# PositronicsLab/Moby

Hardware: AMD Instinct MI355X
Metric: lcp_rows_per_sec (higher is better)
Workload: dtype f64

## Files before the change

moby_amd/csrc/mh_lcp_wave.h:

```cpp
#pragma once
#include "mh_wave.h"
#include "../../include/moby_hip.h"

namespace mh {

enum { LP_SETUP = 0, LP_GATHER, LP_LU, LP_GEMV, LP_RANDMIN, LP_VERIFY, LP_LEMKE, LP_COUNT };
__shared__ unsigned long long g_lcp_prof[LP_COUNT];
__shared__ int g_lcp_prof_on;
#ifdef MH_PROFILE_BUILD
MH_DEV unsigned long long lp_tick() { return g_lcp_prof_on ? __builtin_amdgcn_s_memtime() : 0ull; }
MH_DEV void lp_tock(int ph, unsigned long long t0) { if (g_lcp_prof_on) { const unsigned long long d = __builtin_amdgcn_s_memtime() - t0; if (lane_id() == 0) g_lcp_prof[ph] += d; } }
#else
MH_DEV unsigned long long lp_tick() { return 0ull; }
MH_DEV void lp_tock(int, unsigned long long) {}
#endif

struct Trace {
  int32_t* buf; int cap; int len;
  MH_DEV void push(int32_t v) { if (buf && len < cap && lane_id() == 0) buf[len] = v; len++; }
};

#define MH_DBL_EPS 2.220446049250313e-16
#define MH_NEAR_ZERO 1.4901161193847656e-08
#define MH_SFMIN 2.2250738585072014e-308

struct DenseLds {
  const double* M; int n;
  MH_DEV double at_row(int c) const { const int l = lane_id(); return (l < n) ? M[l + n * c] : 0.0; }
  MH_DEV double diag() const { const int l = lane_id(); return (l < n) ? M[l + n * l] : 0.0; }
  MH_DEV double offdiag_max() const {
    const int lane = lane_id();
    double m = 0.0;
    if (lane < n)
      for (int c = 0; c < n; c++) {
        const double a = fabs(M[lane + n * c]);
        if (c != lane && a > m) m = a;
      }
    return wave_max(m);
  }
};

template <class MatT>
MH_DEV double mat_at(const MatT& M, int c, double lam) {
  const double m = M.at_row(c);
  return (lane_id() == c) ? m + lam : m;
}

MH_DEV int lu_solve_wave(int k, double* A, double& b)
{
  const int lane = lane_id();
  for (int j = 0; j < k; j++) {
    const bool mine = (lane >= j) && (lane < k);
    double a = mine ? fabs(A[lane + k * j]) : -1.0;
    double amax; int jp;
    argmax_first(a, mine, amax, jp);
    if (!(amax != 0.0)) return j + 1;
    if (jp != j) {
      if (lane < k) { double t0 = A[j + k * lane], t1 = A[jp + k * lane]; A[j + k * lane] = t1; A[jp + k * lane] = t0; }
      double bj = read_lane(b, j), bjp = read_lane(b, jp);
      if (lane == j) b = bjp; else if (lane == jp) b = bj;
      wave_sync();
    }
    if (j < k - 1) {
      const double piv = A[j + k * j];
      if (lane > j && lane < k) {
        double l = A[lane + k * j];
        if (fabs(piv) >= MH_SFMIN) { const double r = 1.0 / piv; l = l * r; } else l = l / piv;
        A[lane + k * j] = l;
        for (int c0 = j + 1; c0 < k; c0 += 8) {
          double a[8], u[8];
#pragma unroll
          for (int t = 0; t < 8; t++) {
            const int c = (c0 + t < k) ? c0 + t : k - 1;
            a[t] = A[lane + k * c]; u[t] = A[j + k * c];
          }
#pragma unroll
          for (int t = 0; t < 8; t++)
            if (c0 + t < k) A[lane + k * (c0 + t)] = a[t] - l * u[t];
        }
      }
      wave_sync();
    }
  }
  for (int kk = 0; kk < k; kk++) {
    const double bk = read_lane(b, kk);
    if (lane > kk && lane < k) b = b - bk * A[lane + k * kk];
  }
  for (int kk = k - 1; kk >= 0; kk--) {
    if (lane == kk) b = b / A[kk + k * kk];
    const double bk = read_lane(b, kk);
    if (lane < kk) b = b - bk * A[lane + k * kk];
  }
  return 0;
}

MH_DEV int lu_solve_wave_hbm(int k, double* A, double& b)
{
  constexpr int PB = 8;
  const int lane = lane_id();
  const bool valid = lane < k;
  int prow = lane;
  for (int j0 = 0; j0 < k; j0 += PB) {
    const int nb = (k - j0 < PB) ? k - j0 : PB;
    double p[PB];
#pragma unroll
    for (int c = 0; c < PB; c++) p[c] = (valid && c < nb) ? A[prow + k * (j0 + c)] : 0.0;
#pragma unroll
    for (int jj = 0; jj < PB; jj++) {
      if (jj < nb) {
        const int j = j0 + jj;
        const bool mine = (lane >= j) && valid;
        double amax; int jp;
        argmax_first(mine ? fabs(p[jj]) : -1.0, mine, amax, jp);
        if (!(amax != 0.0)) return j + 1;
        if (jp != j) {
#pragma unroll
          for (int c = 0; c < PB; c++) { const double vj = read_lane(p[c], j), vp = read_lane(p[c], jp); if (lane == j) p[c] = vp; else if (lane == jp) p[c] = vj; }
          { const double vj = read_lane(b, j), vp = read_lane(b, jp); if (lane == j) b = vp; else if (lane == jp) b = vj; }
          { const int rj = read_lane(prow, j), rp = read_lane(prow, jp); if (lane == j) prow = rp; else if (lane == jp) prow = rj; }
        }
        if (j < k - 1) {
          const double piv = read_lane(p[jj], j);
          const bool below = (lane > j) && valid;
          if (below) { double l = p[jj]; if (fabs(piv) >= MH_SFMIN) { const double r = 1.0 / piv; l = l * r; } else l = l / piv; p[jj] = l; }
#pragma unroll
          for (int c = 0; c < PB; c++) if (c > jj && c < nb) { const double u = read_lane(p[c], j); if (below) p[c] = p[c] - p[jj] * u; }
        }
      }
    }
#pragma unroll
    for (int c = 0; c < PB; c++) if (valid && c < nb) A[prow + k * (j0 + c)] = p[c];
    for (int cb = j0 + nb; cb < k; cb += PB) {
      double a[PB];
#pragma unroll
      for (int u = 0; u < PB; u++) a[u] = (valid && cb + u < k) ? A[prow + k * (cb + u)] : 0.0;
#pragma unroll
      for (int u = 0; u < PB; u++) {
#pragma unroll
        for (int s2 = 0; s2 < PB; s2++) if (s2 < nb) { const double us = read_lane(a[u], j0 + s2); if (lane > j0 + s2 && valid) a[u] = a[u] - p[s2] * us; }
      }
#pragma unroll
      for (int u = 0; u < PB; u++) if (valid && cb + u < k) A[prow + k * (cb + u)] = a[u];
    }
  }
  wave_sync();
  for (int kb = 0; kb < k; kb += PB) {
    double l[PB];
#pragma unroll
    for (int u = 0; u < PB; u++) l[u] = (valid && kb + u < k) ? A[prow + k * (kb + u)] : 0.0;
#pragma unroll
    for (int u = 0; u < PB; u++) if (kb + u < k) { const double bk = read_lane(b, kb + u); if (lane > kb + u && valid) b = b - bk * l[u]; }
  }
  for (int ke = k; ke > 0; ke -= PB) {
    const int kb = (ke - PB > 0) ? ke - PB : 0;
    double uu[PB];
#pragma unroll
    for (int u = 0; u < PB; u++) uu[u] = (valid && kb + u < ke) ? A[prow + k * (kb + u)] : 1.0;
#pragma unroll
    for (int u = PB - 1; u >= 0; u--) if (kb + u < ke) {
      const int kk = kb + u;
      if (lane == kk) b = b / uu[u];
      const double bk = read_lane(b, kk);
      if (lane < kk) b = b - bk * uu[u];
    }
  }
  return 0;
}

MH_DEV int rand_min_wave(double v, uint64_t mask, double tol, WaveRand& rng, double& val, bool& tie)
{
  const int lane = lane_id();
  const bool in = (mask >> lane) & 1ull;
  double vmin; int imin;
  if (popc(mask) <= 4) {
    uint64_t m = mask;
    imin = ctz(m); m &= m - 1;
    vmin = read_lane(v, imin);
    while (m) { const int i = ctz(m); m &= m - 1; const double x = read_lane(v, i); if (x < vmin) { vmin = x; imin = i; } }
  } else argmin_first(v, in, vmin, imin);
  const uint64_t qm = ballot(in && lane != imin && v < vmin + tol);
  const int cnt = 1 + popc(qm);
  tie = tie || cnt > 1;
  const int rv = rng.next();
  const int r = (cnt == 1) ? 0 : rv % cnt;
  const int chosen = (r == 0) ? imin : nth_set_bit(qm, r - 1);
  val = read_lane(v, chosen);
  return chosen;
}

MH_DEV double norm_reg(double offmax, double dii, bool valid, double lam) {
  double d = valid ? fabs(dii + lam) : 0.0;
  double m = wave_max(d);
  return (m > offmax) ? m : offmax;
}

struct LuScratch { double* small; int ka; double* big; };

template <int K>
MH_DEV int lu_small(const double* A, double& b)
{
  double a[K][K], x[K];
#pragma unroll
  for (int c = 0; c < K; c++)
#pragma unroll
    for (int r = 0; r < K; r++) a[r][c] = A[r + K * c];
#pragma unroll
  for (int r = 0; r < K; r++) x[r] = read_lane(b, r);
#pragma unroll
  for (int j = 0; j < K; j++) {
    int jp = j; double amax = fabs(a[j][j]);
#pragma unroll
    for (int i = j + 1; i < K; i++) { const double v = fabs(a[i][j]); if (v > amax) { amax = v; jp = i; } }
    jp = uni(jp);
    if (ballot(!(amax != 0.0)) != 0ull) return j + 1;
#pragma unroll
    for (int i = j + 1; i < K; i++)
      if (jp == i) {
#pragma unroll
        for (int c = 0; c < K; c++) { const double t = a[j][c]; a[j][c] = a[i][c]; a[i][c] = t; }
        const double t = x[j]; x[j] = x[i]; x[i] = t;
      }
    if (j < K - 1) {
      const double piv = a[j][j];
      const bool big = fabs(piv) >= MH_SFMIN;
      const double r = 1.0 / piv;
#pragma unroll
      for (int i = j + 1; i < K; i++) {
        const double l = big ? a[i][j] * r : a[i][j] / piv;
        a[i][j] = l;
#pragma unroll
        for (int c = j + 1; c < K; c++) a[i][c] = a[i][c] - l * a[j][c];
      }
    }
  }
#pragma unroll
  for (int kk = 0; kk < K; kk++)
#pragma unroll
    for (int i = kk + 1; i < K; i++) x[i] = x[i] - x[kk] * a[i][kk];
#pragma unroll
  for (int kk = K - 1; kk >= 0; kk--) {
    x[kk] = x[kk] / a[kk][kk];
#pragma unroll
    for (int i = 0; i < kk; i++) x[i] = x[i] - x[kk] * a[i][kk];
  }
  const int lane = lane_id();
  double out = 0.0;
#pragma unroll
  for (int r = 0; r < K; r++) out = (lane == r) ? x[r] : out;
  b = out;
  return 0;
}

#ifndef MH_COLCACHE
#define MH_COLCACHE 4
#endif
template <bool REGLU, class MatT>
MH_DEV int gather_and_solve(const MatT& M, double lam, uint64_t nbmask, int k, bool is_nb, int pos, double qi, double* A, double& b,
                            double (&colv)[MH_COLCACHE])
{
  const int lane = lane_id();
  unsigned long long t0 = lp_tick();
  if (k == 1) {
    const int j = ctz(nbmask);
    const double v = mat_at(M, j, lam);
    colv[0] = v;
    const double a00 = read_lane(v, j);
    const double rhs = read_lane(-qi, j);
    lp_tock(LP_GATHER, t0);
    if (!(fabs(a00) != 0.0)) return 1;
    b = (lane == 0) ? rhs / a00 : 0.0;
    return 0;
  }
  wave_sync();
  uint64_t m = nbmask;
#pragma unroll
  for (int c = 0; c < MH_COLCACHE; c++) {
    if (c < k) {
      const int j = ctz(m); m &= m - 1;
      const double v = mat_at(M, j, lam);
      colv[c] = v;
      if (is_nb) A[pos + k * c] = v;
    }
  }
  for (int c = MH_COLCACHE; c < k; c++) {
    const int j = ctz(m); m &= m - 1;
    const double v = mat_at(M, j, lam);
    if (is_nb) A[pos + k * c] = v;
  }
  b = push_to(-qi, is_nb ? pos : k + popc(~nbmask & lanes_below(lane)));
  wave_sync();
  lp_tock(LP_GATHER, t0);
  t0 = lp_tick();
  int info;
  if (REGLU && k == 2) info = lu_small<2>(A, b);
  else if (REGLU && k == 3) info = lu_small<3>(A, b);
#ifndef MH_NO_LU4
  else if (REGLU && k == 4) info = lu_small<4>(A, b);
#endif
  else info = REGLU ? lu_solve_wave(k, A, b) : lu_solve_wave_hbm(k, A, b);
  lp_tock(LP_LU, t0);
  return info;
}

template <class MatT>
MH_DEV bool lcp_fast_wave(int n, const MatT& M, double lam, LuScratch S,
                          double qi, double& zi, int& zsize, double zero_tol,
                          double nrm_lam, WaveRand& rng, unsigned& pivots, Trace& tr)
{
  const int lane = lane_id();
  const bool valid = lane < n;
  const uint64_t vmask = lanes_below(n);
  if (zero_tol < 0.0) zero_tol = (double)n * nrm_lam * MH_DBL_EPS;
  uint64_t nbmask;
  if (zsize == n) {
    nbmask = ballot(valid && !(fabs(zi) < zero_tol));
  } else {
    double qmin; int minw;
    argmin_first(qi, valid, qmin, minw);
    if (qmin > -zero_tol) { zi = 0.0; zsize = n; pivots = 0; return true; }
    nbmask = bit(minw);
  }
  const unsigned MAX_PIV = 2u * (unsigned)n;
  for (pivots = 0; pivots < MAX_PIV; pivots++) {
    const int k = popc(nbmask);
    const bool is_nb = (nbmask >> lane) & 1ull;
    const bool is_b = valid && !is_nb;
    const int pos = popc(nbmask & lanes_below(lane));
    double b = 0.0;
    double colv[MH_COLCACHE];
    if (k > 0) {
      int info;
      if (k <= S.ka) info = gather_and_solve<true>(M, lam, nbmask, k, is_nb, pos, qi, S.small, b, colv);
      else info = gather_and_solve<false>(M, lam, nbmask, k, is_nb, pos, qi, S.big, b, colv);
      if (info != 0) return false;
    }
    unsigned long long tg = lp_tick();
    double w = 0.0;
    {
      uint64_t m = nbmask;
#pragma unroll
      for (int c = 0; c < MH_COLCACHE; c++) {
        if (c < k) {
          m &= m - 1;
          const double t = read_lane(b, c);
          if (is_b) w = w + t * colv[c];
        }
      }
      for (int c = MH_COLCACHE; c < k; c++) {
        const int j = ctz(m); m &= m - 1;
        const double t = read_lane(b, c);
        const double v = mat_at(M, j, lam);
        if (is_b) w = w + t * v;
      }
      w = w + qi;
    }
    const double zv = __shfl(b, pos);
    lp_tock(LP_GEMV, tg);
    tg = lp_tick();
    const uint64_t bmask = vmask & ~nbmask;
    double wsel = 0.0; int minw = -1;
    bool tie = false;
    if (bmask != 0ull) {
      if (ballot(is_b && !(w > -zero_tol)) == 0ull) (void)rng.next();
      else minw = rand_min_wave(w, bmask, zero_tol, rng, wsel, tie);
    }
    double zsel = 0.0; int minz = -1;
    if (k > 0) {
      if (ballot(is_nb && !(zv >= -zero_tol)) == 0ull) (void)rng.next();
      else minz = rand_min_wave(zv, nbmask, zero_tol, rng, zsel, tie);
    }
    lp_tock(LP_RANDMIN, tg);
    if (minw < 0 || wsel > -zero_tol) {
      if (minz >= 0 && zsel < -zero_tol) {
        nbmask &= ~bit(minz);
        tr.push(-(int32_t)(minz + 1));
      } else {
        zi = is_nb ? zv : 0.0;
        zsize = n;
        return true;
      }
    } else {
      const uint64_t nb_new = nbmask | bit(minw);
      tr.push((int32_t)(minw + 1));
      nbmask = nb_new;
      if (minz >= 0 && zsel < -zero_tol) {
        const int posz = popc((nb_new & ~bit(minw)) & lanes_below(minz));
        const int idx2 = nth_set_bit(nb_new, posz);
        nbmask &= ~bit(idx2);
        tr.push(-(int32_t)(idx2 + 1));
#ifndef MH_NO_REPEAT_SKIP
        if (idx2 == minw && !tie) {
          const unsigned rest = MAX_PIV - (pivots + 1u);
          rng.skip(2u * rest);
          if (tr.buf && tr.len < tr.cap) for (unsigned r = 0; r < rest; r++) { tr.push((int32_t)(minw + 1)); tr.push(-(int32_t)(idx2 + 1)); }
          else tr.len += (int)(2u * rest);
          pivots = MAX_PIV;
          return false;
        }
#endif
      }
    }
  }
  return false;
}

template <class MatT>
MH_DEV bool verify_wave(int n, const MatT& M, double lam, double qi, double zi, double ZERO_TOL, bool strict)
{
  const int lane = lane_id();
  const bool valid = lane < n;
  const double nT = -ZERO_TOL;
  if (ballot(valid && zi != zi) != 0ull) { const double mz = min_element_value(zi, valid); if (!(strict ? (mz > nT) : (mz >= nT))) return false; }
  else if (ballot(valid && !(strict ? (zi > nT) : (zi >= nT))) != 0ull) return false;
  double w = 0.0;
  uint64_t nz = ballot(valid && zi != 0.0);
  while (nz) {
    const int c = ctz(nz); nz &= nz - 1;
    const double t = read_lane(zi, c);
    const double m = mat_at(M, c, lam);
    if (valid) w = w + t * m;
  }
  w = w + qi;
  const double zw = zi * w;
  if (ballot(valid && (w != w || zw != zw)) != 0ull) {
    const double mw = min_element_value(w, valid);
    if (!(strict ? (mw > nT) : (mw >= nT))) return false;
    const double mn = min_element_value(zw, valid), mx = max_element_value(zw, valid);
    return (strict ? (mn > nT) : (mn >= nT)) && mx < ZERO_TOL;
  }
  if (ballot(valid && !(strict ? (w > nT) : (w >= nT))) != 0ull) return false;
  if (ballot(valid && !(strict ? (zw > nT) : (zw >= nT))) != 0ull) return false;
  return ballot(valid && !(zw < ZERO_TOL)) == 0ull;
}

template <bool HBM, class MatT>
MH_DEV int lemke_gather_and_solve(int n, const MatT& M, double lam, int bv, int t, const double* art, double* A, double& d)
{
  const int lane = lane_id();
  const bool valid = lane < n;
  wave_sync();
  for (int p = 0; p < n; p++) {
    const int id = read_lane(bv, p);
    double a;
    if (id == t) a = valid ? art[lane] : 0.0;
    else if (id >= n) a = (lane == id - n) ? -1.0 : 0.0;
    else a = mat_at(M, id, lam);
    if (valid) A[lane + n * p] = a;
  }
  wave_sync();
  return HBM ? lu_solve_wave_hbm(n, A, d) : lu_solve_wave(n, A, d);
}

template <class MatT>
MH_DEV bool lcp_lemke_wave(int n, const MatT& M, double lam, LuScratch S, double* art,
                           double qi, double& zi, int& zsize, double piv_tol, double zero_tol,
                           double nrm_lam, WaveRand& rng, unsigned& pivots, Trace& tr)
{
  const int lane = lane_id();
  const bool valid = lane < n;
  const double INF = __longlong_as_double(0x7ff0000000000000ll);
  const unsigned MAXITER = (50u * (unsigned)n < 1000u) ? 50u * (unsigned)n : 1000u;
  pivots = 0;
  zi = 0.0;
  const int z0size = zsize;
  if (zero_tol <= 0.0) zero_tol = MH_DBL_EPS * nrm_lam * (double)n;
  const double qmin = wave_min(valid ? qi : INF);
  if (qmin > -zero_tol) { zsize = n; return true; }
  zsize = 2 * n;
  const int t = 2 * n;
  if (z0size != n) for (int i = 0; i < n; i++) (void)rng.next();
  int bv = n + lane;
  double x = valid ? qi : 0.0;
  if (ballot(valid && x < 0.0) == 0ull) { zsize = n; return true; }
  const double PIV_TOL = (piv_tol > 0.0) ? piv_tol : MH_DBL_EPS * (double)n * ((nrm_lam > 1.0) ? nrm_lam : 1.0);
  double xmin; int lvindex;
  argmin_first(x, valid, xmin, lvindex);
  const double tval = -xmin;
  int leaving = n + lvindex;
  int entering = t;
  double u = (valid && x < 0.0) ? 1.0 : 0.0;
  wave_sync();
  if (valid) art[lane] = u;
  u = u * tval;
  x = x + u;
  if (lane == lvindex) { x = tval; bv = t; }
  wave_sync();
  for (pivots = 0; pivots < MAXITER; pivots++) {
    if (leaving == t) {
      wave_sync();
      if (valid) art[lane] = 0.0;
      wave_sync();
      if (valid && bv < n) art[bv] = x;
      wave_sync();
      zi = valid ? art[lane] : 0.0;
      zsize = n;
      return true;
    }
    double be;
    if (leaving < n) { entering = n + leaving; be = (lane == leaving) ? -1.0 : 0.0; }
    else { entering = leaving - n; be = valid ? mat_at(M, entering, lam) : 0.0; }
    double d = be;
    {
      int info;
      if (n <= S.ka) info = lemke_gather_and_solve<false>(n, M, lam, bv, t, art, S.small, d);
      else info = lemke_gather_and_solve<true>(n, M, lam, bv, t, art, S.big, d);
      if (info != 0) return false;
    }
    const uint64_t jm = ballot(valid && d > PIV_TOL);
    if (jm == 0ull) return false;
    const bool inj = (jm >> lane) & 1ull;
    const double rat = inj ? (x + zero_tol) / d : INF;
    { const double r0 = read_lane(rat, ctz(jm)); if (r0 != r0) { zsize = n; return false; } }
    const double theta = wave_min(rat);
    const uint64_t keep = ballot(inj && (x / d <= theta));
    if (keep == 0ull) { zsize = n; return false; }
    const uint64_t tm = ballot(valid && bv == t);
    lvindex = (keep & tm) ? ctz(tm) : ctz(keep);
    leaving = read_lane(bv, lvindex);
    const double ratio = read_lane(x, lvindex) / read_lane(d, lvindex);
    d = d * ratio;
    x = x - d;
    if (lane == lvindex) { x = ratio; bv = entering; }
    tr.push((int32_t)entering + 1); tr.push((int32_t)leaving + 1);
  }
  zsize = n;
  return false;
}


struct LcpParams { int kind; int min_exp; unsigned step_exp; int max_exp; double piv_tol; double zero_tol; };

struct Pow10Table { double v[64]; };

template <class MatT>
MH_DEV bool lcp_solve_wave(const LcpParams& P, const Pow10Table& p10, int n, const MatT& M, LuScratch A, double* art,
                           double nrm0, double dii, double qi, double& zi, int& zsize,
                           WaveRand& rng, unsigned& pivots, Trace& tr)
{
  const bool valid = lane_id() < n;
  const bool reg = (P.kind == MH_LCP_FAST_REG) || (P.kind == MH_LCP_LEMKE_REG);
  const bool fast = (P.kind == MH_LCP_FAST) || (P.kind == MH_LCP_FAST_REG);
  const double ZERO_TOL = (P.zero_tol > 0.0) ? P.zero_tol : (double)n * nrm0 * MH_NEAR_ZERO;
  unsigned total = 0;
  double offmax = 0.0;
  int rf = P.min_exp;
  for (int attempt = 0; ; attempt++) {
    double lam = 0.0, nrm = nrm0;
    if (attempt > 0) {
      if (!reg || !(rf < P.max_exp)) break;
      if (attempt == 1) offmax = M.offdiag_max();
      lam = p10.v[rf + 32];
      nrm = norm_reg(offmax, dii, valid, lam);
    }
    if (reg) tr.push(0x40000000 | attempt);
    unsigned long long tl = lp_tick();
    const bool ok = fast ? lcp_fast_wave(n, M, lam, A, qi, zi, zsize, P.zero_tol, nrm, rng, pivots, tr)
                         : lcp_lemke_wave(n, M, lam, A, art, qi, zi, zsize, P.piv_tol, P.zero_tol, nrm, rng, pivots, tr);
    if (!fast) lp_tock(LP_LEMKE, tl);
    if (!reg) return ok;
    tl = lp_tick();
    const bool good = ok && verify_wave(n, M, lam, qi, zi, ZERO_TOL, attempt > 0);
    lp_tock(LP_VERIFY, tl);
    if (attempt == 0) { if (good) return true; total += pivots; }
    else { total += pivots; if (good) { pivots = total; return true; } rf += (int)P.step_exp; }
  }
  pivots = total;
  return false;
}

}
```

moby_amd/csrc/mh_world_wave.inc:

```
#include "mh_world_common.h"

#define MHW_CAT_(a, b) a##b
#define MHW_CAT(a, b) MHW_CAT_(a, b)
#if defined(MH_PROFILE_BUILD)
#define MHW_NS MHW_CAT(MHW_BASE, _prof)
#elif defined(MH_FORCES_BUILD)
#define MHW_NS MHW_CAT(MHW_BASE, _forces)
#define MHW_FORCES 1
#else
#define MHW_NS MHW_BASE
#endif
#define MHW_VARIANT_GETTER MHW_CAT(mh_world_variant_, MHW_NS)

#define MHW_NS_MAXC ((MHW_MAX_CONTACTS < 6) ? MHW_MAX_CONTACTS : 6)
#define MHW_KA_V ((12 * MHW_MAX_ROWS >= 256) ? 16 : 12)
#define MHW_NS_MAXM (2 * MHW_NS_MAXC)

namespace mh { namespace MHW_NS {

enum {
  D_ST = 0,
  D_QSAVE = D_ST + 13 * MHW_NB,
  D_VSAVE = D_QSAVE + 7 * MHW_NB,
  D_QV = D_VSAVE + 6 * MHW_NB,
  D_DQV = D_QV + 7 * MHW_NB,
  D_XINV = D_DQV + 7 * MHW_NB,
  D_XQ = D_XINV + 10 * MHW_NB,
  D_JW = D_XQ + 4 * MHW_NB,
  D_CPT = D_JW + 9 * MHW_NB,
  D_CNR = D_CPT + 3 * MHW_MAX_CONTACTS,
  D_CS1 = D_CNR + 3 * MHW_MAX_CONTACTS,
  D_CS2 = D_CS1 + 3 * MHW_MAX_CONTACTS,
  D_CDIST = D_CS2 + 3 * MHW_MAX_CONTACTS,
  D_CMU = D_CDIST + MHW_MAX_CONTACTS,
  D_CMUV = D_CMU + MHW_MAX_CONTACTS,
  D_CEPS = D_CMUV + MHW_MAX_CONTACTS,
  D_CCOMP = D_CEPS + MHW_MAX_CONTACTS,
  D_J = D_CCOMP + MHW_MAX_CONTACTS,
  D_XJ = D_J + 12 * MHW_MAX_ROWS,
  D_G = D_XJ + 12 * MHW_MAX_ROWS,
  D_CV = D_G + MHW_MAX_GROWS * MHW_MAX_GROWS,
  D_IMP = D_CV + MHW_MAX_ROWS,
  D_A = D_J,
  D_ART = D_IMP + MHW_MAX_ROWS,
  D_ZLAST = D_ART + 64,
  D_ZBUF = D_ZLAST + 64,
  D_ZSOL = D_ZBUF,
  D_RADIUS = D_ZBUF + 64,
  D_RMAX = D_RADIUS + MHW_NB,
  D_GDIM = D_RMAX + MHW_NB,
  D_MASS = D_GDIM + (MHW_BOX ? 3 * MHW_NB : 0),
  D_INERTIA = D_MASS + MHW_NB,
  D_PLANE_R = D_INERTIA + 3 * MHW_NB,
  D_PLANE_O = D_PLANE_R + 9,
  D_GRAV = D_PLANE_O + 3,
  D_PMU = D_GRAV + 3,
  D_PMUV = D_PMU + MHW_MAX_PAIRS,
  D_PEPS = D_PMUV + MHW_MAX_PAIRS,
  D_PCOMP = D_PEPS + MHW_MAX_PAIRS,
  D_MINSTEP = D_PCOMP + MHW_MAX_PAIRS,
  D_THRESH = D_MINSTEP + 1,
  D_CSTABEPS = D_THRESH + 1,
  D_TIME = D_CSTABEPS + 1,
  D_SPK = D_TIME + 1,
  D_VNS = D_SPK + (MHW_NOSLIP ? 2 * MH_MAX_SPOKES : 0),
  D_NSY = D_VNS + (MHW_NOSLIP ? MH_NOSLIP_MAX : 0),
  D_NSQX = D_NSY + (MHW_NOSLIP ? MHW_NS_MAXM * MHW_NS_MAXM : 0),
  D_NSW = D_NSQX + (MHW_NOSLIP ? MHW_NS_MAXC * MHW_NS_MAXM : 0),
  D_NSMM = D_NSW + (MHW_NOSLIP ? MHW_NS_MAXC * MHW_NS_MAXM : 0),
  D_NSQ = D_NSMM + (MHW_NOSLIP ? MHW_NS_MAXC * MHW_NS_MAXC : 0),
  D_NSYXV = D_NSQ + (MHW_NOSLIP ? MHW_NS_MAXC : 0),
  D_NST2 = D_NSYXV + (MHW_NOSLIP ? MHW_NS_MAXM : 0),
  D_END = D_NST2 + (MHW_NOSLIP ? MHW_NS_MAXM : 0)
};
enum {
  I_PAIRS = 0,
  I_CG1 = I_PAIRS + MHW_MAX_PAIRS,
  I_CG2 = I_CG1 + MHW_MAX_CONTACTS,
  I_CPAIR = I_CG2 + MHW_MAX_CONTACTS,
  I_CNK = I_CPAIR + MHW_MAX_CONTACTS,
  I_ROWOFF = I_CNK + MHW_MAX_CONTACTS,
  I_ISLC = I_ROWOFF + 2 * MHW_MAX_ROWS,
  I_ISLB = I_ISLC + MHW_MAX_CONTACTS,
  I_KOFF = I_ISLB + MHW_NB,
  I_SCR = I_KOFF + MHW_MAX_CONTACTS + 1,
  I_RNG = I_SCR + 64,
  I_PNK = I_RNG + 32,
  I_PEN = I_PNK + MHW_MAX_PAIRS,
  I_NB = I_PEN + MHW_MAX_PAIRS, I_NTOT, I_NPT, I_NMAX, I_KA, I_NPAIRS, I_NC, I_STATUS,
  I_ZLAST_SIZE, I_ZBUF_SIZE, I_ZBUF_CAP, I_NODEMASK, I_DONEMASK, I_DONEMASK_HI, I_CSTAB_MAXIT,
  I_NSPOKES, I_VNS_SIZE, I_NSM, I_NSNS,
  I_GEOM,
  I_NSS = I_GEOM + MHW_NB,
  I_NST = I_NSS + (MHW_NOSLIP ? MHW_NS_MAXC : 0),
  I_END = I_NST + (MHW_NOSLIP ? MHW_NS_MAXC : 0)
};
__shared__ double gd[D_END];
__shared__ int gi[I_END];
__shared__ double* g_lu_ws;

enum { CN_STEPS = 0, CN_MINI, CN_LCP, CN_ROWS, CN_PIV, CN_STAB, CN_BYTES, CN_SROWS, CN_COUNT };
enum { PH_BROAD_CA = 0, PH_INTEGRATE, PH_FWDDYN, PH_CONTACTS, PH_ISLANDS, PH_PDATA, PH_MBUILD, PH_LCP, PH_APPLY, PH_STAB,
       PH_LP0, PH_COUNT = PH_LP0 + LP_COUNT };
__shared__ unsigned long long g_cnt[CN_COUNT];
__shared__ unsigned long long g_pacc[PH_COUNT];
#if MHW_FORCES
enum { F_SB = 0, F_SBA = MHW_NB, F_KL = 2 * MHW_NB, F_KA = 3 * MHW_NB, F_KLSQ = 4 * MHW_NB, F_KASQ = 5 * MHW_NB, F_WR = 6 * MHW_NB, F_END = 12 * MHW_NB };
#define MHW_FORCE_WRENCH 0x100
__shared__ double gf[F_END];
__shared__ int g_fterms;
#endif

#if MHW_STATICS
enum { S_R = 0, S_O = 9 * MH_MAX_STATICS, S_DIM = 12 * MH_MAX_STATICS, S_RAD = 15 * MH_MAX_STATICS, S_END = 16 * MH_MAX_STATICS };
__shared__ double gs[S_END];
__shared__ int gst[MH_MAX_STATICS];
#endif

#if MHW_REPORT
__shared__ double g_racc[3 * MHW_MAX_CONTACTS];
__shared__ double* g_rep;
#endif

#define MHW_FN __device__ __noinline__

MH_DEV int geti(int i) { return uni(gi[i]); }
MH_DEV void seti(int i, int v) { if (lane_id() == 0) gi[i] = v; }
#ifdef MH_PROFILE_BUILD
MH_DEV unsigned long long tick() { return g_lcp_prof_on ? __builtin_amdgcn_s_memtime() : 0ull; }
MH_DEV void tock(int ph, unsigned long long t0) { if (g_lcp_prof_on) { const unsigned long long d = __builtin_amdgcn_s_memtime() - t0; if (lane_id() == 0) g_pacc[ph] += d; } }
#else
MH_DEV unsigned long long tick() { return 0ull; }
MH_DEV void tock(int, unsigned long long) {}
#endif
MH_DEV void account(int n, unsigned piv) {
  if (lane_id() == 0) { g_cnt[CN_LCP]++; g_cnt[CN_ROWS] += (unsigned long long)n; g_cnt[CN_PIV] += piv; g_cnt[CN_BYTES] += 8ull * ((unsigned long long)n * n + 2ull * n); }
}

MH_DEV bool enabled(int b) { return b < gi[I_NB]; }
MH_DEV V3 X(int b) { return v3(gd[D_ST + 13*b], gd[D_ST + 13*b+1], gd[D_ST + 13*b+2]); }
MH_DEV V3 Vl(int b) { return v3(gd[D_ST + 13*b+7], gd[D_ST + 13*b+8], gd[D_ST + 13*b+9]); }
MH_DEV V3 Wa(int b) { return v3(gd[D_ST + 13*b+10], gd[D_ST + 13*b+11], gd[D_ST + 13*b+12]); }
MH_DEV V3 point_vel(int b, V3 p) {
  if (!enabled(b)) return v3(0.0, 0.0, 0.0);
  return Vl(b) + cross(Wa(b), p - X(b));
}
MH_DEV void pair_bodies(int p, int& a, int& b) {
  const int ntot = gi[I_NTOT];
  int i = 0, rem = p;
  while (rem >= ntot - 1 - i) { rem -= ntot - 1 - i; i++; }
  a = i; b = i + 1 + rem;
}
#if MHW_STATICS
MH_DEV const double* plane_R(int pl) { return gs + S_R + 9 * (pl - gi[I_NB]); }
MH_DEV const double* plane_o(int pl) { return gs + S_O + 3 * (pl - gi[I_NB]); }
#define plane_body(pl) (pl)
#else
MH_DEV const double* plane_R(int) { return gd + D_PLANE_R; }
MH_DEV const double* plane_o(int) { return gd + D_PLANE_O; }
#define plane_body(pl) gi[I_NB]
#endif
MH_DEV V3 plane_n(int pl) { const double* R = plane_R(pl); return v3(R[1], R[4], R[7]); }
MH_DEV V3 to_plane(V3 p, int pl) {
  const double* R = plane_R(pl); const double* o = plane_o(pl); V3 d = p - v3(o[0], o[1], o[2]);
  return v3((R[0]*d.x + R[3]*d.y) + R[6]*d.z, (R[1]*d.x + R[4]*d.y) + R[7]*d.z, (R[2]*d.x + R[5]*d.y) + R[8]*d.z);
}
MH_DEV V3 from_plane(V3 p, int pl) {
  const double* R = plane_R(pl); const double* o = plane_o(pl);
  return v3(o[0] + ((R[0]*p.x + R[1]*p.y) + R[2]*p.z),
            o[1] + ((R[3]*p.x + R[4]*p.y) + R[5]*p.z),
            o[2] + ((R[6]*p.x + R[7]*p.y) + R[8]*p.z));
}
MH_DEV void orthonormal_basis(V3 n, V3& s, V3& t) {
  const double ax = fabs(n.x), ay = fabs(n.y), az = fabs(n.z);
  V3 e;
  if (ax <= ay && ax <= az) e = v3(1.0, 0.0, 0.0); else if (ay <= az) e = v3(0.0, 1.0, 0.0); else e = v3(0.0, 0.0, 1.0);
  s = cross(n, e); s = s / norm(s);
  t = cross(n, s);
}

MH_DEV void rot(int b, double R[9]) {
  const double x = gd[D_ST + 13*b+3], y = gd[D_ST + 13*b+4], z = gd[D_ST + 13*b+5], w = gd[D_ST + 13*b+6];
  R[0] = 1.0 - 2.0 * (y*y + z*z); R[1] = 2.0 * (x*y - z*w);       R[2] = 2.0 * (x*z + y*w);
  R[3] = 2.0 * (x*y + z*w);       R[4] = 1.0 - 2.0 * (x*x + z*z); R[5] = 2.0 * (y*z - x*w);
  R[6] = 2.0 * (x*z - y*w);       R[7] = 2.0 * (y*z + x*w);       R[8] = 1.0 - 2.0 * (x*x + y*y);
}
MH_DEV bool is_spokes(int b) {
#if MHW_NOSLIP
  return b < gi[I_NB] && gi[I_GEOM + b] == MH_GEOM_SPOKES;
#else
  (void)b; return false;
#endif
}
#if MHW_NOSLIP
MH_DEV V3 spoke_tip_at(const double R[9], V3 c, int i) {
  const double px = gd[D_SPK + 2*i], py = 0.0, pz = gd[D_SPK + 2*i + 1];
  return v3(c.x + ((R[0]*px + R[1]*py) + R[2]*pz), c.y + ((R[3]*px + R[4]*py) + R[5]*pz), c.z + ((R[6]*px + R[7]*py) + R[8]*pz));
}
MH_DEV V3 spoke_tip(int b, int i) { double R[9]; rot(b, R); return spoke_tip_at(R, X(b), i); }
#endif

MH_DEV bool is_box(int b) {
#if MHW_BOX
  return b < gi[I_NB] && gi[I_GEOM + b] == MH_GEOM_BOX;
#else
  (void)b; return false;
#endif
}
#if MHW_BOX
MH_DEV V3 box_corner(int b, int i) {
  const double hx = gd[D_GDIM + 3*b] * 0.5, hy = gd[D_GDIM + 3*b + 1] * 0.5, hz = gd[D_GDIM + 3*b + 2] * 0.5;
  return v3((i & 4) ? -hx : hx, (i & 2) ? -hy : hy, (i & 1) ? -hz : hz);
}
MH_DEV V3 box_vertex(int b, int i) {
  const V3 p = box_corner(b, i);
  double R[9]; rot(b, R);
  const V3 c = X(b);
  return v3(c.x + ((R[0]*p.x + R[1]*p.y) + R[2]*p.z), c.y + ((R[3]*p.x + R[4]*p.y) + R[5]*p.z), c.z + ((R[6]*p.x + R[7]*p.y) + R[8]*p.z));
}
MH_DEV unsigned box_contact_mask(int b, double TOL, int pl) {
  unsigned m = 0;
  for (int i = 0; i < 8; i++) { const V3 pp = to_plane(box_vertex(b, i), pl); if (pp.y <= TOL) m |= 1u << i; }
  return m;
}
MH_DEV bool rel_equal(double x, double y) {
  const double ax = fabs(x), ay = fabs(y);
  const double m1 = (ay > 1.0) ? ay : 1.0; const double m = (ax > m1) ? ax : m1;
  return fabs(x - y) <= MH_NEAR_ZERO * m;
}
MH_DEV bool collinear(V3 a, V3 b, V3 c) {
  return rel_equal((c.z-a.z)*(b.y-a.y), (b.z-a.z)*(c.y-a.y)) && rel_equal((b.z-a.z)*(c.x-a.x), (b.x-a.x)*(c.z-a.z)) &&
         rel_equal((b.x-a.x)*(c.y-a.y), (b.y-a.y)*(c.x-a.x));
}
#endif
#if MHW_BSP
MH_DEV bool is_sphere(int b) { return b < gi[I_NB] && gi[I_GEOM + b] == MH_GEOM_SPHERE; }
#if MHW_STATICS
MH_DEV bool is_static(int b, int type) { const int s = b - gi[I_NB]; return s >= 0 && s < MH_MAX_STATICS && b < gi[I_NTOT] && gst[s] == type; }
MH_DEV bool is_ground(int b) { return is_static(b, MH_STATIC_PLANE); }
MH_DEV bool is_sbox(int b) { return is_static(b, MH_STATIC_BOX); }
#else
MH_DEV bool is_ground(int b) { return b == gi[I_NB]; }
MH_DEV bool is_sbox(int) { return false; }
#endif
MH_DEV bool bsp_pair(int a, int b, int& bx, int& sp) {
  if (is_box(a) && is_sphere(b)) { bx = a; sp = b; return true; }
  if (is_sphere(a) && (is_box(b) || is_sbox(b))) { bx = b; sp = a; return true; }
  return false;
}
MH_DEV void box_frame(int bx, double R[9], V3& cb, V3& h) {
#if MHW_STATICS
  if (bx >= gi[I_NB]) {
    const int s = bx - gi[I_NB];
#pragma unroll
    for (int k = 0; k < 9; k++) R[k] = gs[S_R + 9*s + k];
    cb = v3(gs[S_O + 3*s], gs[S_O + 3*s + 1], gs[S_O + 3*s + 2]);
    h = v3(gs[S_DIM + 3*s] * 0.5, gs[S_DIM + 3*s + 1] * 0.5, gs[S_DIM + 3*s + 2] * 0.5);
    return;
  }
#endif
  rot(bx, R); cb = X(bx);
  h = v3(gd[D_GDIM + 3*bx] * 0.5, gd[D_GDIM + 3*bx + 1] * 0.5, gd[D_GDIM + 3*bx + 2] * 0.5);
}
MH_DEV V3 mat_v(const double R[9], V3 p) { return v3((R[0]*p.x + R[1]*p.y) + R[2]*p.z, (R[3]*p.x + R[4]*p.y) + R[5]*p.z, (R[6]*p.x + R[7]*p.y) + R[8]*p.z); }
MH_DEV V3 matT_v(const double R[9], V3 p) { return v3((R[0]*p.x + R[3]*p.y) + R[6]*p.z, (R[1]*p.x + R[4]*p.y) + R[7]*p.z, (R[2]*p.x + R[5]*p.y) + R[8]*p.z); }
MH_DEV double clampd(double c, double h) { return (c < -h) ? -h : ((c > h) ? h : c); }
MH_DEV int bsp_contact(int bx, int sp, double TOL, V3& pt, V3& n, double& dist) {
  double R[9]; V3 cb, h; box_frame(bx, R, cb, h);
  const V3 cS = X(sp);
  const V3 c = matT_v(R, cS - cb);
  const double Rs = gd[D_RADIUS + sp];
  const V3 p = v3(clampd(c.x, h.x), clampd(c.y, h.y), clampd(c.z, h.z));
  V3 u = p - c;
  const double nrm = norm(u);
  if (fabs(p.x) < h.x || fabs(p.y) < h.y || fabs(p.z) < h.z || nrm < Rs) {
    const double b1 = h.y - fabs(p.y), b2 = h.z - fabs(p.z);
    const double b12 = (b2 < b1) ? b2 : b1, b0 = h.x - fabs(p.x);
    const double bd = (b12 < b0) ? b12 : b0;
    const double rn = Rs - nrm;
    dist = -((rn < bd) ? rn : bd);
  } else {
    u = u * (Rs / nrm);
    dist = norm((c + u) - p);
  }
  if (dist > TOL) return 0;
  const V3 ug = mat_v(R, u);
  const V3 sg = cS + ug;
  bool own = false;
  if (dist > 0.0) {
    const V3 pg = cb + mat_v(R, p);
    const V3 nd = pg - sg;
    const double nl = norm(nd);
    pt = (sg + pg) * 0.5;
    if (nl > MH_NEAR_ZERO) { n = nd / nl; own = true; }
  } else pt = sg;
  if (!own) n = ug / norm(ug);
  return 1;
}
MH_DEV double bsp_sdist(int bx, int sp, V3& pA, V3& pB) {
  double R[9]; V3 cb, hv; box_frame(bx, R, cb, hv);
  const V3 cS = X(sp);
  const V3 cv = matT_v(R, cS - cb);
  const double c[3] = { cv.x, cv.y, cv.z };
  const double h[3] = { hv.x, hv.y, hv.z };
  const double Rs = gd[D_RADIUS + sp];
  double cl[3] = { c[0], c[1], c[2] };
  bool inside = true; double sq = 0.0, in = -MHW_INF;
#pragma unroll
  for (int i = 0; i < 3; i++) {
    if (c[i] < -h[i]) { const double dl = c[i] + h[i]; cl[i] = -h[i]; sq = sq + dl * dl; inside = false; }
    else if (c[i] > h[i]) { const double dl = c[i] - h[i]; cl[i] = h[i]; sq = sq + dl * dl; inside = false; }
    else if (inside) { const double f1 = fabs(h[i] - c[i]), f2 = fabs(c[i] + h[i]); const double dd = -((f2 < f1) ? f2 : f1); in = (in < dd) ? dd : in; }
  }
  const double dist = (inside ? in : sqrt(sq)) - Rs;
  const V3 v = v3(cl[0] - c[0], cl[1] - c[1], cl[2] - c[2]);
  const double vn = norm(v);
  pA = cb + mat_v(R, v3(cl[0], cl[1], cl[2]));
  if (vn == 0.0) pB = cS;
  else pB = cS + mat_v(R, v) * ((Rs + ((0.0 < dist) ? 0.0 : dist)) / vn);
  return dist;
}
#endif
#if MHW_BSP
#define box_plane_pair(a, b) (is_box(a) && is_ground(b))
#else
#define box_plane_pair(a, b) is_box(a)
#endif

MH_DEV void bounds(int b, double dt, V3& lo, V3& hi) {
#if MHW_STATICS
  if (is_sbox(b)) {
    const int s = b - gi[I_NB];
    const V3 c = v3(gs[S_O + 3*s], gs[S_O + 3*s + 1], gs[S_O + 3*s + 2]); const double r = gs[S_RAD + s];
    lo = v3(c.x - r, c.y - r, c.z - r); hi = v3(c.x + r, c.y + r, c.z + r); return;
  }
#endif
  if (!enabled(b)) { lo = v3(-MHW_INF, -MHW_INF, -MHW_INF); hi = v3(MHW_INF, MHW_INF, MHW_INF); return; }
  const V3 c = X(b);
  const V3 vdt = Vl(b) * dt, wdt = Wa(b) * dt;
  const V3 lin = vdt + cross(c, wdt);
  const V3 p2 = c + lin;
  const double r = gd[D_RADIUS + b];
  lo = v3(((c.x < p2.x) ? c.x : p2.x) - r, ((c.y < p2.y) ? c.y : p2.y) - r, ((c.z < p2.z) ? c.z : p2.z) - r);
  hi = v3(((c.x > p2.x) ? c.x : p2.x) + r, ((c.y > p2.y) ? c.y : p2.y) + r, ((c.z > p2.z) ? c.z : p2.z) + r);
}
MHW_FN int broad_phase(double dt, int out_off) {
  const int lane = lane_id();
  bool keep = false, spk = false;
  if (lane < gi[I_NPT]) {
    int a, b; pair_bodies(lane, a, b);
    if (is_spokes(a) || is_spokes(b)) {
      spk = true; keep = is_spokes(a) && b == gi[I_NB];
#if MHW_BSP
    } else if (is_box(a) && (is_box(b) || is_sbox(b))) {
      keep = false;
#else
    } else if ((is_box(a) || is_box(b)) && b != gi[I_NB]) {
      keep = false;
#endif
    } else {
      V3 loa, hia, lob, hib; bounds(a, dt, loa, hia); bounds(b, dt, lob, hib);
      keep = (loa.x <= hib.x && lob.x <= hia.x) && (loa.y <= hib.y && lob.y <= hia.y) && (loa.z <= hib.z && lob.z <= hia.z);
      keep = keep && (gi[I_PEN + lane] != 0) && (enabled(a) || enabled(b));
    }
  }
  const uint64_t m = ballot(keep && !spk);
  const uint64_t ms = ballot(keep && spk);
  wave_sync();
  if (keep) gi[out_off + (spk ? popc(m) + popc(ms & lanes_below(lane)) : popc(m & lanes_below(lane)))] = lane;
  wave_sync();
  return popc(m) + popc(ms);
}
struct PairGeom { double dist; V3 pa, pb; int a, b; };
MHW_FN PairGeom pair_geom(int p) {
  PairGeom g; pair_bodies(p, g.a, g.b);
#if MHW_NOSLIP
  if (is_spokes(g.a)) {
    const int w = g.a, N = gi[I_NSPOKES];
    double min_dist = MHW_INF;
    g.pa = v3(0.0, 0.0, 0.0); g.pb = v3(0.0, 0.0, 0.0);
    double Rw[9]; rot(w, Rw);
    const V3 cw = X(w);
    for (int i = 0; i < N; i++) {
      const V3 tip = spoke_tip_at(Rw, cw, i);
      const V3 pp = to_plane(tip, gi[I_NB]);
      if (pp.y < min_dist) { min_dist = pp.y; g.pb = from_plane(v3(pp.x, 0.0, pp.z), gi[I_NB]); g.pa = tip; }
    }
    g.dist = min_dist; g.a = gi[I_NB]; g.b = w;
    return g;
  }
#endif
#if MHW_BSP
  { int bx, sp;
    if (bsp_pair(g.a, g.b, bx, sp)) {
      V3 pbox, psph; g.dist = bsp_sdist(bx, sp, pbox, psph);
      if (bx == g.a) { g.pa = pbox; g.pb = psph; } else { g.pa = psph; g.pb = pbox; }
      return g;
    } }
#endif
#if MHW_BOX
  if (is_box(g.a)) {
    double min_dist = MHW_INF;
    g.pa = v3(0.0, 0.0, 0.0); g.pb = v3(0.0, 0.0, 0.0);
    for (int i = 0; i < 8; i++) {
      const V3 vtx = box_vertex(g.a, i);
      const V3 pp = to_plane(vtx, g.b);
      if (pp.y < min_dist) { min_dist = pp.y; g.pa = vtx; g.pb = from_plane(v3(pp.x, 0.0, pp.z), g.b); }
    }
    g.dist = min_dist;
    return g;
  }
#endif
  if (enabled(g.a) && enabled(g.b)) {
    const V3 ca = X(g.a), cb = X(g.b);
    const double ra = gd[D_RADIUS + g.a], rb = gd[D_RADIUS + g.b];
    const V3 ab = cb - ca;
    const double len = norm(ab);
    const double d = len - ra - rb;
    const V3 u = ab / len;
    const double sa = (d > 0.0) ? ra : ra + d, sb = (d > 0.0) ? rb : rb + d;
    g.pa = ca + u * sa; g.pb = cb - u * sb; g.dist = d;
    return g;
  }
  const int s = enabled(g.a) ? g.a : g.b, pl = enabled(g.a) ? g.b : g.a;
  const V3 cp = to_plane(X(s), pl);
  const double r = gd[D_RADIUS + s];
  const double low = cp.y + (-1.0 * r);
  const V3 on_plane = from_plane(v3(cp.x, 0.0, cp.z), pl);
  const V3 on_sphere = from_plane(v3(cp.x, low, cp.z), pl);
  if (s == g.a) { g.pa = on_sphere; g.pb = on_plane; } else { g.pa = on_plane; g.pb = on_sphere; }
  g.dist = low;
  return g;
}
struct ContactGeom { int has, g1, g2; V3 pt, n; double dist; };
struct ContactGeomPacked { int code; V3 pt, n; double dist; };
MH_DEV ContactGeom contact_geom_body(int p, double TOL);
MHW_FN ContactGeomPacked contact_geom_packed(int p, double TOL) {
  const ContactGeom c = contact_geom_body(p, TOL);
  ContactGeomPacked q; q.code = c.has | (c.g1 << 8) | (c.g2 << 16); q.pt = c.pt; q.n = c.n; q.dist = c.dist;
  return q;
}
MH_DEV ContactGeom contact_geom(int p, double TOL) {
  const ContactGeomPacked q = contact_geom_packed(p, TOL);
  ContactGeom c; c.has = q.code & 0xff; c.g1 = (q.code >> 8) & 0xff; c.g2 = (q.code >> 16) & 0xff; c.pt = q.pt; c.n = q.n; c.dist = q.dist;
  return c;
}
MH_DEV ContactGeom contact_geom_body(int p, double TOL) {
  ContactGeom c; c.has = 0; c.g1 = 0; c.g2 = 0; c.pt = v3(0.0, 0.0, 0.0); c.n = v3(0.0, 0.0, 0.0); c.dist = 0.0;
  int a, b; pair_bodies(p, a, b);
#if MHW_BSP
  { int bx, sp;
    if (bsp_pair(a, b, bx, sp)) {
      c.has = bsp_contact(bx, sp, TOL, c.pt, c.n, c.dist); c.g1 = bx; c.g2 = sp;
      return c;
    } }
#endif
  if (enabled(a) && enabled(b)) {
    const V3 cA = X(a), cB = X(b);
    const double rA = gd[D_RADIUS + a], rB = gd[D_RADIUS + b];
    const V3 d = cA - cB;
    const double len = norm(d);
    c.dist = len - rA - rB;
    if (c.dist > TOL) return c;
    c.n = d / len;
    const V3 closest_A = cA - c.n * rA, closest_B = cB + c.n * rB;
    c.pt = (closest_A + closest_B) * 0.5;
    c.g1 = a; c.g2 = b; c.has = 1;
    return c;
  }
  const int s = enabled(a) ? a : b, pl = enabled(a) ? b : a;
  const V3 cp = to_plane(X(s), pl);
  const double r = gd[D_RADIUS + s];
  c.dist = cp.y - r;
  if (c.dist > TOL) return c;
  c.pt = from_plane(v3(cp.x, 0.5 * (cp.y - r), cp.z), pl);
  c.n = plane_n(pl); c.g1 = s; c.g2 = pl; c.has = 1;
  return c;
}
MH_DEV double rel_vel(int g1, int g2, V3 pt, V3 dir) { return dot(dir, point_vel(g1, pt) - point_vel(g2, pt)); }
MH_DEV double calc_max_dist(int b, V3 n, double rmax) {
  if (!enabled(b)) return 0.0;
  const V3 xd0 = Vl(b) + cross(X(b), Wa(b));
  return dot(n, xd0) + norm(cross(Wa(b), n)) * rmax;
}
MH_DEV double ca_step(int p) {
  const PairGeom g = pair_geom(p);
  ContactGeom c; c.has = 0;
  bool have_c = false;
  if (is_spokes(g.b)) {
    if (g.dist <= 0.0) return MHW_INF;
  } else
#if MHW_BOX
  if (box_plane_pair(g.a, g.b)) {
    if (g.dist <= 0.0) {
      const unsigned m = box_contact_mask(g.a, MH_NEAR_ZERO, g.b);
      if (m == 0u) return MHW_INF;
      const V3 cn = -plane_n(g.b);
      const int gnd = plane_body(g.b);
      V3 p3[3]; int np = 0; V3 first = v3(0.0, 0.0, 0.0);
      for (int i = 0; i < 8; i++) if ((m >> i) & 1u) {
        const V3 vtx = box_vertex(g.a, i);
        if (rel_vel(gnd, g.a, vtx, cn) < -MH_NEAR_ZERO) return 0.0;
        if (np == 0) first = vtx;
        if (np < 3) p3[np] = vtx;
        np++;
      }
      if (np >= 3 && !collinear(p3[0], p3[1], p3[2])) return MHW_INF;
      const V3 normal = -cn; const double offset0 = -dot(cn, first);
      double R[9]; rot(g.a, R);
      const V3 nP = v3((R[0]*normal.x + R[3]*normal.y) + R[6]*normal.z, (R[1]*normal.x + R[4]*normal.y) + R[7]*normal.z, (R[2]*normal.x + R[5]*normal.y) + R[8]*normal.z);
      const V3 dp = normal * offset0 - X(g.a);
      const V3 dpb = v3((R[0]*dp.x + R[3]*dp.y) + R[6]*dp.z, (R[1]*dp.x + R[4]*dp.y) + R[7]*dp.z, (R[2]*dp.x + R[5]*dp.y) + R[8]*dp.z);
      const double offset = dot(nP, dpb);
      const V3 w = Wa(g.a), vl = Vl(g.a);
      const V3 wb = v3((R[0]*w.x + R[3]*w.y) + R[6]*w.z, (R[1]*w.x + R[4]*w.y) + R[7]*w.z, (R[2]*w.x + R[5]*w.y) + R[8]*w.z);
      const V3 vb = v3((R[0]*vl.x + R[3]*vl.y) + R[6]*vl.z, (R[1]*vl.x + R[4]*vl.y) + R[7]*vl.z, (R[2]*vl.x + R[5]*vl.y) + R[8]*vl.z);
      const double av_norm = norm(wb);
      const double lv_dot_n = -dot(nP, vb);
      double max_step = MHW_INF;
      for (int i = 0; i < 8; i++) {
        const V3 vtx = box_corner(g.a, i);
        const double r = norm(vtx);
        const double dist = dot(nP, vtx) - offset;
        if (dist < MH_NEAR_ZERO) continue;
        const double sp = lv_dot_n + av_norm * r;
        const double speed = (0.0 > sp) ? 0.0 : sp;
        const double cand = dist / speed;
        max_step = (cand < max_step) ? cand : max_step;
      }
      return max_step;
    }
  } else
#endif
  if (!(g.dist > MH_NEAR_ZERO)) {
    c = contact_geom(p, MH_NEAR_ZERO); have_c = true;
    if (c.has && fabs(rel_vel(c.g1, c.g2, c.pt, c.n)) < MH_NEAR_ZERO * 10) return MHW_INF;
  }
  if (g.dist <= 0.0 && !is_spokes(g.b) && !box_plane_pair(g.a, g.b)) {
    if (!have_c) c = contact_geom(p, MH_NEAR_ZERO);
    if (!c.has) return MHW_INF;
    if (rel_vel(c.g1, c.g2, c.pt, c.n) < -MH_NEAR_ZERO) return 0.0;
    return MHW_INF;
  }
  const V3 d0 = g.pa - g.pb;
  const V3 n0 = d0 / norm(d0);
  const double tA = calc_max_dist(g.a, -n0, enabled(g.a) ? gd[D_RMAX + g.a] : 0.0);
  const double tB = calc_max_dist(g.b, n0, enabled(g.b) ? gd[D_RMAX + g.b] : 0.0);
  double total = tA + tB;
  if (total < 0.0) total = 0.0;
  const double cand = g.dist / total;
  return (cand < MHW_INF) ? cand : MHW_INF;
}

MH_DEV void inertia_world(int b, double Jw[9]) {
  double R[9]; rot(b, R);
  double T[9];
#pragma unroll
  for (int i = 0; i < 3; i++)
#pragma unroll
    for (int j = 0; j < 3; j++) T[3*i+j] = R[3*i+j] * gd[D_INERTIA + 3*b + j];
#pragma unroll
  for (int i = 0; i < 3; i++)
#pragma unroll
    for (int j = 0; j < 3; j++) Jw[3*i+j] = (T[3*i] * R[3*j] + T[3*i+1] * R[3*j+1]) + T[3*i+2] * R[3*j+2];
  Jw[1] = Jw[3]; Jw[2] = Jw[6]; Jw[5] = Jw[7];
}
MHW_FN void compute_xinv() {
  const int lane = lane_id();
  wave_sync();
  bool stale = false;
  if (lane < gi[I_NB]) {
#pragma unroll
    for (int k = 0; k < 4; k++) stale = stale || !(gd[D_XQ + 4*lane + k] == gd[D_ST + 13*lane + 3 + k]);
  }
  if (ballot(stale) == 0ull) return;
  if (stale) {
    const int b = lane;
#pragma unroll
    for (int k = 0; k < 4; k++) gd[D_XQ + 4*b + k] = gd[D_ST + 13*b + 3 + k];
    double im;
    { const double l = sqrt(gd[D_MASS + b]); const double e = 1.0 / l; im = e / l; }
    double Jw[9]; inertia_world(b, Jw);
#pragma unroll
    for (int k = 0; k < 9; k++) gd[D_JW + 9*b + k] = Jw[k];
    double l00, l10, l20, l11, l21, l22;
    { double ajj = Jw[0]; ajj = sqrt(ajj); l00 = ajj; l10 = Jw[3] / ajj; l20 = Jw[6] / ajj; }
    { double ajj = Jw[4]; ajj = ajj - l10 * l10; ajj = sqrt(ajj); l11 = ajj; double s = Jw[7]; s = s - l20 * l10; l21 = s / ajj; }
    { double ajj = Jw[8]; ajj = ajj - l20 * l20; ajj = ajj - l21 * l21; ajj = sqrt(ajj); l22 = ajj; }
    double col[3][3];
#pragma unroll
    for (int c = 0; c < 3; c++) {
      double b0 = (c == 0) ? 1.0 : 0.0, b1 = (c == 1) ? 1.0 : 0.0, b2 = (c == 2) ? 1.0 : 0.0;
      b0 = b0 / l00; b1 = b1 - b0 * l10; b2 = b2 - b0 * l20;
      b1 = b1 / l11; b2 = b2 - b1 * l21;
      b2 = b2 / l22;
      { double s = b2; b2 = s / l22; }
      { double s = b1; s = s - l21 * b2; b1 = s / l11; }
      { double s = b0; s = s - l10 * b1; s = s - l20 * b2; b0 = s / l00; }
      col[c][0] = b0; col[c][1] = b1; col[c][2] = b2;
    }
    double Ai[9];
#pragma unroll
    for (int c = 0; c < 3; c++)
#pragma unroll
      for (int i = 0; i < 3; i++) Ai[i + 3*c] = col[c][i];
    Ai[0 + 3*1] = Ai[1 + 3*0]; Ai[0 + 3*2] = Ai[2 + 3*0]; Ai[1 + 3*2] = Ai[2 + 3*1];
    gd[D_XINV + 10*b] = im;
#pragma unroll
    for (int r = 0; r < 3; r++)
#pragma unroll
      for (int c = 0; c < 3; c++) gd[D_XINV + 10*b + 1 + 3*r + c] = Ai[r + 3*c];
  }
  wave_sync();
}
MH_DEV void euler_vel(int b, double qd[7]) {
  const V3 v = Vl(b), w = Wa(b);
  const double x = gd[D_ST + 13*b+3], y = gd[D_ST + 13*b+4], z = gd[D_ST + 13*b+5], ww = gd[D_ST + 13*b+6];
  qd[0] = v.x; qd[1] = v.y; qd[2] = v.z;
  qd[3] = 0.5 * ((ww * w.x + z * w.y) - y * w.z);
  qd[4] = 0.5 * ((ww * w.y + x * w.z) - z * w.x);
  qd[5] = 0.5 * ((ww * w.z + y * w.x) - x * w.y);
  qd[6] = 0.5 * (((-x * w.x) - y * w.y) - z * w.z);
}
MH_DEV void set_coords(int b, const double q[7]) {
  gd[D_ST + 13*b] = q[0]; gd[D_ST + 13*b+1] = q[1]; gd[D_ST + 13*b+2] = q[2];
  const double nrm = sqrt(((q[3]*q[3] + q[4]*q[4]) + q[5]*q[5]) + q[6]*q[6]);
  gd[D_ST + 13*b+3] = q[3] / nrm; gd[D_ST + 13*b+4] = q[4] / nrm; gd[D_ST + 13*b+5] = q[5] / nrm; gd[D_ST + 13*b+6] = q[6] / nrm;
}
MHW_FN void set_q_from(int base_off, int dq_off, double t, int scale) {
  const int lane = lane_id();
  wave_sync();
  if (lane < gi[I_NB]) {
    double q[7];
#pragma unroll
    for (int k = 0; k < 7; k++) { double v = gd[dq_off + 7*lane + k]; if (scale) v = v * t; q[k] = v + gd[base_off + 7*lane + k]; }
    set_coords(lane, q);
  }
  wave_sync();
}
MH_DEV void integrate_positions(double hh) {
  const int lane = lane_id();
  wave_sync();
  if (lane < gi[I_NB]) {
    set_coords(lane, gd + D_QSAVE + 7 * lane);
    double qd[7]; euler_vel(lane, qd);
    double q[7];
#pragma unroll
    for (int i = 0; i < 7; i++) { q[i] = qd[i] * hh; q[i] = q[i] + gd[D_QSAVE + 7*lane + i]; }
    set_coords(lane, q);
  }
  wave_sync();
}
#if MHW_FORCES
MH_DEV void integrate_velocities_forced(double h, int ft) {
  const int lane = lane_id();
  compute_xinv();
  if (lane < gi[I_NB]) {
    const int b = lane;
    const double m = gd[D_MASS + b];
    V3 F = v3(gd[D_GRAV] * m, gd[D_GRAV + 1] * m, gd[D_GRAV + 2] * m);
    V3 T = v3(0.0, 0.0, 0.0);
    bool has_t = false;
    const V3 v = Vl(b), w = Wa(b);
    if (ft & MH_FORCE_STOKES) {
      F = F + v * (-gf[F_SB + b]);
      T = w * (-gf[F_SBA + b]); has_t = true;
    }
    if (ft & MH_FORCE_DAMPING) {
      double R[9]; rot(b, R);
      const V3 vi = v3((R[0]*v.x + R[3]*v.y) + R[6]*v.z, (R[1]*v.x + R[4]*v.y) + R[7]*v.z, (R[2]*v.x + R[5]*v.y) + R[8]*v.z);
      const V3 wi = v3((R[0]*w.x + R[3]*w.y) + R[6]*w.z, (R[1]*w.x + R[4]*w.y) + R[7]*w.z, (R[2]*w.x + R[5]*w.y) + R[8]*w.z);
      const V3 fb = vi * (-(gf[F_KL + b] + norm(vi) * gf[F_KLSQ + b]));
      const V3 tb = wi * (-(gf[F_KA + b] + norm(wi) * gf[F_KASQ + b]));
      const V3 fw = v3((R[0]*fb.x + R[1]*fb.y) + R[2]*fb.z, (R[3]*fb.x + R[4]*fb.y) + R[5]*fb.z, (R[6]*fb.x + R[7]*fb.y) + R[8]*fb.z);
      const V3 tw = v3((R[0]*tb.x + R[1]*tb.y) + R[2]*tb.z, (R[3]*tb.x + R[4]*tb.y) + R[5]*tb.z, (R[6]*tb.x + R[7]*tb.y) + R[8]*tb.z);
      F = F + fw;
      T = has_t ? T + tw : tw; has_t = true;
    }
    if (ft & MHW_FORCE_WRENCH) {
      const double* r = gf + F_WR + 6*b;
      F = F + v3(r[0], r[1], r[2]);
      const V3 tq = v3(r[3], r[4], r[5]);
      T = has_t ? T + tq : tq; has_t = true;
    }
    const V3 xdd = F / m;
    const double* Jw = gd + D_JW + 9*b;
    const V3 Jww = v3((Jw[0]*w.x + Jw[1]*w.y) + Jw[2]*w.z, (Jw[3]*w.x + Jw[4]*w.y) + Jw[5]*w.z, (Jw[6]*w.x + Jw[7]*w.y) + Jw[8]*w.z);
    const V3 tau = has_t ? T - cross(w, Jww) : -cross(w, Jww);
    const double* Ji = gd + D_XINV + 10*b + 1;
    const V3 wd = v3((Ji[0]*tau.x + Ji[1]*tau.y) + Ji[2]*tau.z, (Ji[3]*tau.x + Ji[4]*tau.y) + Ji[5]*tau.z, (Ji[6]*tau.x + Ji[7]*tau.y) + Ji[8]*tau.z);
    const V3 vn = v + xdd * h, wn = w + wd * h;
    gd[D_ST + 13*b+7] = vn.x; gd[D_ST + 13*b+8] = vn.y; gd[D_ST + 13*b+9] = vn.z;
    gd[D_ST + 13*b+10] = wn.x; gd[D_ST + 13*b+11] = wn.y; gd[D_ST + 13*b+12] = wn.z;
  }
  wave_sync();
}
#endif
MH_DEV void integrate_velocities(double h) {
#if MHW_FORCES
  { const int ft = uni(g_fterms); if (ft != 0) { integrate_velocities_forced(h, ft); return; } }
#endif
  const int lane = lane_id();
  compute_xinv();
  if (lane < gi[I_NB]) {
    const int b = lane;
    const double m = gd[D_MASS + b];
    const V3 f = v3(gd[D_GRAV] * m, gd[D_GRAV + 1] * m, gd[D_GRAV + 2] * m);
    const V3 xdd = f / m;
    const double* Jw = gd + D_JW + 9*b;
    const V3 w = Wa(b);
    const V3 Jww = v3((Jw[0]*w.x + Jw[1]*w.y) + Jw[2]*w.z, (Jw[3]*w.x + Jw[4]*w.y) + Jw[5]*w.z, (Jw[6]*w.x + Jw[7]*w.y) + Jw[8]*w.z);
    const V3 tau = -cross(w, Jww);
    const double* Ji = gd + D_XINV + 10*b + 1;
    const V3 wd = v3((Ji[0]*tau.x + Ji[1]*tau.y) + Ji[2]*tau.z, (Ji[3]*tau.x + Ji[4]*tau.y) + Ji[5]*tau.z, (Ji[6]*tau.x + Ji[7]*tau.y) + Ji[8]*tau.z);
    const V3 vn = Vl(b) + xdd * h, wn = w + wd * h;
    gd[D_ST + 13*b+7] = vn.x; gd[D_ST + 13*b+8] = vn.y; gd[D_ST + 13*b+9] = vn.z;
    gd[D_ST + 13*b+10] = wn.x; gd[D_ST + 13*b+11] = wn.y; gd[D_ST + 13*b+12] = wn.z;
  }
  wave_sync();
}

MHW_FN void store_contact(int slot, int p, int g1, int g2, V3 pt, V3 n, double dist) {
  V3 s, t; orthonormal_basis(n, s, t);
  gi[I_CG1 + slot] = g1; gi[I_CG2 + slot] = g2; gi[I_CPAIR + slot] = p; gi[I_CNK + slot] = gi[I_PNK + p];
  gd[D_CPT + 3*slot] = pt.x; gd[D_CPT + 3*slot+1] = pt.y; gd[D_CPT + 3*slot+2] = pt.z;
  gd[D_CNR + 3*slot] = n.x; gd[D_CNR + 3*slot+1] = n.y; gd[D_CNR + 3*slot+2] = n.z;
  gd[D_CS1 + 3*slot] = s.x; gd[D_CS1 + 3*slot+1] = s.y; gd[D_CS1 + 3*slot+2] = s.z;
  gd[D_CS2 + 3*slot] = t.x; gd[D_CS2 + 3*slot+1] = t.y; gd[D_CS2 + 3*slot+2] = t.z;
  gd[D_CDIST + slot] = dist; gd[D_CMU + slot] = gd[D_PMU + p]; gd[D_CMUV + slot] = gd[D_PMUV + p];
  gd[D_CEPS + slot] = gd[D_PEPS + p]; gd[D_CCOMP + slot] = gd[D_PCOMP + p];
}
MH_DEV V3 Cpt(int i) { return v3(gd[D_CPT + 3*i], gd[D_CPT + 3*i+1], gd[D_CPT + 3*i+2]); }
MH_DEV V3 Cdir(int i, int d) {
  const int o = (d == 0) ? D_CNR : (d == 1 ? D_CS1 : D_CS2);
  return v3(gd[o + 3*i], gd[o + 3*i+1], gd[o + 3*i+2]);
}
MH_DEV double contact_vn(int i) { return rel_vel(gi[I_CG1 + i], gi[I_CG2 + i], Cpt(i), Cdir(i, 0)); }

#if MHW_NOSLIP
MHW_FN int spoke_contacts(int p, int nc) {
  p = uni(p); nc = uni(nc);
  const int lane = lane_id();
  int a, b; pair_bodies(p, a, b);
  bool has = false; V3 pt = v3(0.0, 0.0, 0.0); double dist = 0.0;
  if (lane < gi[I_NSPOKES]) {
    const V3 tip = spoke_tip(a, lane);
    const V3 pp = to_plane(tip, b);
    has = pp.y < gd[D_THRESH];
    pt = (tip + from_plane(v3(pp.x, 0.0, pp.z), b)) * 0.5;
    dist = pp.y;
  }
  const uint64_t m = ballot(has);
  wave_sync();
  if (nc + popc(m) > MHW_MAX_CONTACTS) { seti(I_STATUS, geti(I_STATUS) | MH_WORLD_UNSUPPORTED); wave_sync(); return nc; }
  if (has) store_contact(nc + popc(m & lanes_below(lane)), p, a, b, pt, plane_n(b), dist);
  wave_sync();
  return nc + popc(m);
}
#endif

#if MHW_BOX
MHW_FN int gen_contacts(int list_off, int count, int mode) {
  list_off = uni(list_off); count = uni(count); mode = uni(mode);
  const int lane = lane_id();
  const double thresh = gd[D_THRESH];
  ContactGeom c; c.has = 0; c.g1 = 0; c.g2 = 0; c.pt = v3(0, 0, 0); c.n = v3(0, 0, 0); c.dist = 0.0;
  int p = 0, cnt = 0, bx = -1; unsigned bmask = 0u;
  int bpl = 0;
  if (lane < count) {
    p = gi[list_off + lane];
    const PairGeom g = pair_geom(p);
    if (is_spokes(g.b)) { }
    else if (mode == 1 && g.dist >= MH_NEAR_ZERO) {
      const V3 nn = g.pb - g.pa;
      c.n = nn / norm(nn); c.pt = g.pa; c.g1 = g.a; c.g2 = g.b; c.dist = g.dist; c.has = 1; cnt = 1;
    } else if (mode == 1 || g.dist < thresh) {
      const double TOL = (mode == 1) ? MH_NEAR_ZERO : thresh;
      if (box_plane_pair(g.a, g.b)) { bx = g.a; bpl = g.b; bmask = box_contact_mask(bx, TOL, bpl); cnt = popc((uint64_t)bmask); }
      else { c = contact_geom(p, TOL); cnt = c.has; }
    }
  }
  int off = 0, total = 0;
  { uint64_t m = ballot(cnt > 0);
    while (m) { const int k = ctz(m); m &= m - 1; const int ck = read_lane(cnt, k); if (lane > k) off += ck; total += ck; } }
  wave_sync();
  if (total > MHW_MAX_CONTACTS) return -1;
  if (bx >= 0) {
    const V3 cn = -plane_n(bpl); const int gnd = plane_body(bpl);
    for (int i = 0; i < 8; i++) if ((bmask >> i) & 1u) {
      const V3 vtx = box_vertex(bx, i);
      store_contact(off, p, gnd, bx, vtx, cn, to_plane(vtx, bpl).y);
      off++;
    }
  } else if (c.has) store_contact(off, p, c.g1, c.g2, c.pt, c.n, c.dist);
  wave_sync();
  return total;
}
#endif

MH_DEV void islands_begin() {
  const int lane = lane_id();
  const int nc = geti(I_NC), nb = geti(I_NB);
  const bool in = lane < nc;
  const int a = in ? gi[I_CG1 + lane] : -1, b = in ? gi[I_CG2 + lane] : -1;
  unsigned nodes = 0;
  for (int k = 0; k < nb; k++) if (ballot(in && (a == k || b == k)) != 0ull) nodes |= 1u << k;
  wave_sync();
  seti(I_NODEMASK, (int)nodes); seti(I_DONEMASK, 0); seti(I_DONEMASK_HI, 0);
  wave_sync();
}
MH_DEV int next_island() {
  const int lane = lane_id();
  const int nc = geti(I_NC);
  unsigned node_mask = (unsigned)geti(I_NODEMASK);
  uint64_t done = (uint64_t)(unsigned)geti(I_DONEMASK) | ((uint64_t)(unsigned)geti(I_DONEMASK_HI) << 32);
  const bool in = lane < nc;
  const int a = in ? gi[I_CG1 + lane] : -1, b = in ? gi[I_CG2 + lane] : -1;
  const uint64_t both = ballot(in && enabled(a) && enabled(b));
  int result = -1;
  wave_sync();
  while (node_mask) {
    const int start = __ffs((int)node_mask) - 1;
    unsigned visited = 1u << start, bodies = 0;
    uint64_t queue = (uint64_t)start; int qlen = 1;
    int nic = 0;
    while (qlen > 0) {
      const int nd = (int)(queue & 15ull); queue >>= 4; qlen--;
      node_mask &= ~(1u << nd);
      bodies |= 1u << nd;
      const uint64_t touch = ballot(in && (a == nd || b == nd));
      uint64_t m = touch & both;
      while (m) {
        const int i = ctz(m); m &= m - 1;
        const int ai = read_lane(a, i), bi = read_lane(b, i);
        const int nbr = (ai == nd) ? bi : ai;
        if (!((visited >> nbr) & 1u)) { visited |= 1u << nbr; queue |= (uint64_t)nbr << (4 * qlen); qlen++; }
      }
      const uint64_t fresh = touch & ~done;
      if ((fresh >> lane) & 1ull) gi[I_ISLC + nic + popc(fresh & lanes_below(lane))] = lane;
      nic += popc(fresh);
      done |= fresh;
    }
    if (nic == 0) continue;
    if (lane < 32 && ((bodies >> lane) & 1u)) gi[I_ISLB + popc((uint64_t)(bodies & ((1u << lane) - 1u)))] = lane;
    result = nic | (popc((uint64_t)bodies) << 8);
    break;
  }
  wave_sync();
  seti(I_NODEMASK, (int)node_mask); seti(I_DONEMASK, (int)(unsigned)done); seti(I_DONEMASK_HI, (int)(unsigned)(done >> 32));
  wave_sync();
  return result;
}

MH_DEV int gc_of(int body, int nib) { for (int k = 0; k < nib; k++) if (gi[I_ISLB + k] == body) return 6 * k; return -1; }
MH_DEV void compute_problem_data(int nic, int nib, int ndir, int fresh_xinv) {
  nic = uni(nic); nib = uni(nib); ndir = uni(ndir); fresh_xinv = uni(fresh_xinv);
  const int lane = lane_id();
  const int R = ndir * nic;
  if (fresh_xinv) compute_xinv();
  if (lane < R) {
    const int d = small_div(lane, nic), i = lane - d * nic;
    const int ci = gi[I_ISLC + i];
    const V3 dir = Cdir(ci, d), pt = Cpt(ci);
    double cv = 0.0;
#pragma unroll
    for (int k = 0; k < 2; k++) {
      const int b = (k == 0) ? gi[I_CG1 + ci] : gi[I_CG2 + ci];
      double* Jr = gd + D_J + 12 * lane + 6 * k; double* XJr = gd + D_XJ + 12 * lane + 6 * k;
      if (!enabled(b)) { gi[I_ROWOFF + 2*lane + k] = -1; continue; }
      const V3 dd = (k == 0) ? dir : -dir;
      const V3 r = pt - X(b);
      const V3 rxd = cross(r, dd);
      gi[I_ROWOFF + 2*lane + k] = gc_of(b, nib);
      Jr[0] = dd.x; Jr[1] = dd.y; Jr[2] = dd.z; Jr[3] = rxd.x; Jr[4] = rxd.y; Jr[5] = rxd.z;
      const double im = gd[D_XINV + 10*b]; const double* Ji = gd + D_XINV + 10*b + 1;
      XJr[0] = dd.x * im; XJr[1] = dd.y * im; XJr[2] = dd.z * im;
#pragma unroll
      for (int c = 0; c < 3; c++) XJr[3 + c] = (rxd.x * Ji[c] + rxd.y * Ji[3 + c]) + rxd.z * Ji[6 + c];
      const V3 vl = Vl(b), wa = Wa(b);
      double tmp = 0.0;
      tmp = tmp + dd.x * vl.x; tmp = tmp + dd.y * vl.y; tmp = tmp + dd.z * vl.z;
      tmp = tmp + rxd.x * wa.x; tmp = tmp + rxd.y * wa.y; tmp = tmp + rxd.z * wa.z;
      cv = cv + tmp;
    }
    gd[D_CV + lane] = cv;
  }
  wave_sync();
  {
    const unsigned mnic = small_div_magic(nic), mR = small_div_magic(R);
    for (int e = lane; e < R * R; e += 64) {
      int r = small_div_m(e, mR), c = e - r * R;
      if (small_div_m(c, mnic) < small_div_m(r, mnic)) { const int t = r; r = c; c = t; }
      double res = 0.0;
#pragma unroll
      for (int k = 0; k < 2; k++) {
        const int off = gi[I_ROWOFF + 2*r + k];
        if (off < 0) continue;
        double tmp = 0.0;
        int kk = -1;
        if (gi[I_ROWOFF + 2*c] == off) kk = 0; else if (gi[I_ROWOFF + 2*c + 1] == off) kk = 1;
        if (kk >= 0) {
          const double* Jr = gd + D_J + 12 * r + 6 * k; const double* XJc = gd + D_XJ + 12 * c + 6 * kk;
#pragma unroll
          for (int q = 0; q < 6; q++) tmp = tmp + Jr[q] * XJc[q];
        }
        res = res + tmp;
      }
      gd[D_G + e] = res;
    }
  }
  wave_sync();
}

struct WorldMat {
  int mode, nic, R, nvars, n, doff; unsigned mnic;
  int rkind, ra, ri, grow, gcol, rneg, rvar;
  double rmu, rcos, rsin, rcomp;
  MH_DEV static int dir_of(int a) { return (a == 0) ? 0 : ((a == 1 || a == 3) ? 1 : 2); }
  MH_DEV void init(int mode_, int nic_, int n_) {
    mode = mode_; nic = nic_; n = n_;
    doff = (mode == 2) ? (int)D_NSMM : (int)D_G;
    R = (mode == 0) ? 3 * nic_ : nic_; nvars = 5 * nic_; mnic = 0u;
    const int r = lane_id();
    rkind = 3; ra = 0; ri = 0; grow = 0; gcol = 0; rneg = 0; rvar = 0; rmu = 0.0; rcos = 0.0; rsin = 0.0; rcomp = 0.0;
    if (mode != 0) return;
    mnic = small_div_magic(nic);
    if (r < nvars) { rkind = 0; rvar = 1; ra = small_div_m(r, mnic); ri = r - ra * nic; }
    else if (r < nvars + nic) { rkind = 0; ra = 0; ri = r - nvars; }
    else if (r < n) {
      rkind = 2;
      const int rr = r - nvars - nic;
      int i = 0; while (rr >= gi[I_KOFF + i + 1]) i++;
      ri = i; const int rj = rr - gi[I_KOFF + i];
      const int ci = gi[I_ISLC + i]; const int kh = gi[I_CNK + ci] / 2;
      rmu = gd[D_CMU + ci]; rcos = c_fric.c[kh][rj]; rsin = c_fric.s[kh][rj];
    }
    if (rkind == 0) {
      rcomp = gd[D_CCOMP + gi[I_ISLC + ri]];
      gcol = dir_of(ra) * nic + ri; grow = D_G + gcol * R; rneg = (ra >= 3) ? 1 : 0;
    }
  }
  MH_DEV double at_row(int c) const {
    if (mode != 0) { const int l = lane_id(); return (l < n) ? gd[doff + l * n + c] : 0.0; }
    if (c < nvars) {
      const int b = small_div_m(c, mnic), j = c - b * nic;
      const int bneg = (b >= 3) ? 1 : 0;
      if (rkind == 0) {
        double g = gd[grow + dir_of(b) * nic + j];
        if (rneg != bneg) g = -g;
        if (ra == 0 && b == 0 && ri == j) g = g + rcomp;
        return g;
      }
      if (rkind == 2 && j == ri) return (b == 0) ? rmu : ((b == 1 || b == 3) ? -rcos : -rsin);
      return 0.0;
    }
    if (!rvar) return 0.0;
    const int cc = c - nvars;
    if (cc < nic) {
      double g = gd[D_G + cc * R + gcol];
      if (rneg) g = -g;
      if (ra == 0 && ri == cc) g = g + rcomp;
      return -g;
    }
    int i = 0; const int rr = cc - nic; while (rr >= gi[I_KOFF + i + 1]) i++;
    if (i != ri) return -0.0;
    const int jj = rr - gi[I_KOFF + i]; const int ci = gi[I_ISLC + i]; const int kh = gi[I_CNK + ci] / 2;
    const double v = (ra == 0) ? gd[D_CMU + ci] : ((ra == 1 || ra == 3) ? -c_fric.c[kh][jj] : -c_fric.s[kh][jj]);
    return -v;
  }
  MH_DEV double diag() const {
    if (mode != 0) { const int l = lane_id(); return (l < n) ? gd[doff + l * n + l] : 0.0; }
    if (!rvar) return 0.0;
    double g = gd[grow + gcol];
    if (ra == 0) g = g + rcomp;
    return g;
  }
  MH_DEV double norm_all() const {
    const int lane = lane_id();
    double m = 0.0;
    if (mode != 0) {
      if (lane < n) for (int c = 0; c < n; c++) { const double a = fabs(gd[doff + lane * n + c]); m = (a > m) ? a : m; }
      return wave_max(m);
    }
    for (int e = lane; e < R * R; e += 64) {
      const int r = small_div(e, R), c = e - r * R;
      double g = gd[D_G + e];
      if (r == c && r < nic) g = g + gd[D_CCOMP + gi[I_ISLC + r]];
      const double a = fabs(g); m = (a > m) ? a : m;
    }
    if (lane < nic) { const double a = fabs(gd[D_CMU + gi[I_ISLC + lane]]); m = (a > m) ? a : m; }
    m = wave_max(m);
    return (m > 1.0) ? m : 1.0;
  }
  MH_DEV double offdiag_max() const {
    if (mode != 0) {
      const int lane = lane_id(); double m = 0.0;
      if (lane < n) for (int c = 0; c < n; c++) { const double a = fabs(gd[doff + lane * n + c]); if (c != lane && a > m) m = a; }
      return wave_max(m);
    }
    return norm_all();
  }
};

struct ChainOut { int ok; double zi; int zsize; unsigned piv; };
MH_DEV ChainOut world_lcp_chain(int mode, int nic, int n, double qi, double zi, int zsize)
{
  mode = uni(mode); nic = uni(nic); n = uni(n); zsize = uni(zsize);
  const int lane = lane_id();
  const unsigned long long ts = lp_tick();
  WorldMat M; M.init(mode, nic, n);
  const double nrm0 = M.norm_all(), dii = M.diag();
  lp_tock(LP_SETUP, ts);
  WaveRand rng; rng.r = (lane < 31) ? (unsigned)gi[I_RNG + lane] : 0u; rng.idx = geti(I_RNG + 31);
  LuScratch S; S.small = gd + D_A; S.ka = geti(I_KA);
  S.big = reinterpret_cast<double*>(uni((uint64_t)reinterpret_cast<uintptr_t>(g_lu_ws)));
  Trace tr; tr.buf = nullptr; tr.cap = 0; tr.len = 0;
  unsigned ptot = 0;
  bool ok = false;
  for (int stage = 0; stage < 2; stage++) {
    LcpParams P; P.piv_tol = -1.0; P.zero_tol = -1.0; P.min_exp = -20;
    if (stage == 0) {
      if (mode == 0) { P.kind = MH_LCP_FAST_REG; P.step_exp = 4; P.max_exp = -8; }
      else { P.kind = MH_LCP_FAST; P.step_exp = 1; P.max_exp = 1; }
    } else {
      if (mode == 0) zi = 0.0;
      P.kind = MH_LCP_LEMKE_REG; P.step_exp = 1; P.max_exp = 1;
    }
    unsigned piv = 0;
    ok = lcp_solve_wave(P, c_pow10, n, M, S, gd + D_ART, nrm0, dii, qi, zi, zsize, rng, piv, tr);
    ptot += piv;
    if (ok) break;
  }
  wave_sync();
  if (lane < 31) gi[I_RNG + lane] = (int)rng.r;
  if (lane == 31) gi[I_RNG + 31] = rng.idx;
  wave_sync();
  ChainOut o; o.ok = ok ? 1 : 0; o.zi = zi; o.zsize = zsize; o.piv = ptot;
  return o;
}

MH_DEV int solve_impact_lcp(int nic) {
  nic = uni(nic);
  const int lane = lane_id();
  wave_sync();
  if (lane == 0) { int acc = 0; for (int i = 0; i < nic; i++) { gi[I_KOFF + i] = acc; acc += gi[I_CNK + gi[I_ISLC + i]] / 2; } gi[I_KOFF + nic] = acc; }
  wave_sync();
  const int nk_total = geti(I_KOFF + nic);
  const int nvars = 5 * nic, n = nvars + nic + nk_total;
  if (n > geti(I_NMAX) || n > MH_LCP_MAX_N_WAVE) { seti(I_STATUS, geti(I_STATUS) | MH_WORLD_UNSUPPORTED); wave_sync(); return 0; }
  unsigned long long tm = tick();
  double qi = 0.0;
  if (lane < n) {
    const int r = lane;
    if (r < nvars) { const int a = small_div(r, nic), i = r - a * nic; const double v = gd[D_CV + WorldMat::dir_of(a) * nic + i]; qi = (a >= 3) ? -v : v; }
    else if (r < nvars + nic) qi = gd[D_CV + r - nvars];
    else {
      int i = 0; const int rr = r - nvars - nic; while (rr >= gi[I_KOFF + i + 1]) i++;
      const double cs = gd[D_CV + nic + i], ct = gd[D_CV + 2 * nic + i];
      const double vel = sqrt(cs * cs + ct * ct);
      qi = gd[D_CMUV + gi[I_ISLC + i]] * vel;
    }
  }
  tock(PH_MBUILD, tm);
  tm = tick();
  const int zbuf_cap = geti(I_ZBUF_CAP), zlast_size = geti(I_ZLAST_SIZE);
  double zi;
  if (n > zbuf_cap) zi = 0.0; else zi = gd[D_ZBUF + lane];
  if (lane >= n) zi = 0.0;
  if (n == zlast_size) zi = (lane < n) ? gd[D_ZLAST + lane] : 0.0;
  const ChainOut co = world_lcp_chain(0, nic, n, qi, zi, n);
  zi = co.zi;
  const bool ok = uni(co.ok) != 0;
  account(n, uni(co.piv));
  tock(PH_LCP, tm);
  if (!ok) { seti(I_STATUS, geti(I_STATUS) | MH_WORLD_LCP_FAILED); wave_sync(); return -1; }
  wave_sync();
  if (lane < n) { gd[D_ZLAST + lane] = zi; gd[D_ZBUF + lane] = zi; }
  seti(I_ZLAST_SIZE, n);
  if (zbuf_cap < n) seti(I_ZBUF_CAP, n);
  seti(I_ZBUF_SIZE, 5 * nic);
  wave_sync();
  return 1;
}

MHW_FN void apply_impulses(int nic, int nib, int ndir) {
  nic = uni(nic); nib = uni(nib); ndir = uni(ndir);
  const int lane = lane_id();
  wave_sync();
  const int ngc = 6 * nib;
  if (lane < ngc) {
    const int bi = lane / 6, k = lane - 6 * bi;
    double dv = 0.0;
    for (int d = 0; d < ndir; d++) {
      double tmp = 0.0;
      for (int j = 0; j < nic; j++) {
        const int r = d * nic + j;
        const double t = gd[D_IMP + r];
        int kk = -1;
        if (gi[I_ROWOFF + 2*r] == 6 * bi) kk = 0; else if (gi[I_ROWOFF + 2*r + 1] == 6 * bi) kk = 1;
        if (kk >= 0) tmp = tmp + t * gd[D_XJ + 12 * r + 6 * kk + k];
      }
      if (d == 0) dv = tmp; else dv = dv + tmp;
    }
    const int b = gi[I_ISLB + bi];
    gd[D_ST + 13*b + 7 + k] = gd[D_ST + 13*b + 7 + k] + dv;
  }
#if MHW_REPORT
  if (ndir == 3 && lane < nic) {
    const int ci = gi[I_ISLC + lane];
    for (int d = 0; d < 3; d++) g_racc[3*ci + d] = g_racc[3*ci + d] + gd[D_IMP + d * nic + lane];
  }
#endif
  wave_sync();
}
MH_DEV double Gab3(int R, int nic, int a, int b, int i, int j) {
  return gd[D_G + (a * nic + i) * R + (b * nic + j)];
}
MH_DEV void update_constraint_vels(int nic) {
  nic = uni(nic);
  const int lane = lane_id();
  const int R = 3 * nic;
  double cv = 0.0;
  if (lane < R) {
    const int a = small_div(lane, nic), i = lane - a * nic;
    cv = gd[D_CV + lane];
    for (int b = 0; b < 3; b++) {
      double t = 0.0;
      for (int j = 0; j < nic; j++) t = t + gd[D_IMP + b * nic + j] * Gab3(R, nic, a, b, i, j);
      cv = cv + t;
    }
  }
  wave_sync();
  if (lane < R) gd[D_CV + lane] = cv;
  wave_sync();
}
MH_DEV void impulses_from_z_and_apply(int nic, int nib) {
  nic = uni(nic);
  const int lane = lane_id();
  wave_sync();
  if (lane < nic) {
    const int i = lane;
    gd[D_IMP + i] = gd[D_ZSOL + i];
    double s = gd[D_ZSOL + nic + i];   s = s - gd[D_ZSOL + 3 * nic + i]; gd[D_IMP + nic + i] = s;
    double t = gd[D_ZSOL + 2 * nic + i]; t = t - gd[D_ZSOL + 4 * nic + i]; gd[D_IMP + 2 * nic + i] = t;
  }
  wave_sync();
  apply_impulses(nic, nib, 3);
}
MH_DEV double min_cnv(int nic) { const int lane = lane_id(); return wave_min((lane < nic) ? gd[D_CV + lane] : MHW_INF); }

MH_DEV bool apply_model(int nic, int nib) {
  nic = uni(nic); nib = uni(nib);
  const int lane = lane_id();
  if (3 * nic > MHW_MAX_ROWS) { seti(I_STATUS, geti(I_STATUS) | MH_WORLD_UNSUPPORTED); wave_sync(); return false; }
  unsigned long long t0 = tick();
  compute_problem_data(nic, nib, 3, 0);
  tock(PH_PDATA, t0);
  double minv = 0.0;
  for (int pass = 0; pass < 2; pass++) {
    { const int rs = solve_impact_lcp(nic); if (rs <= 0) return rs < 0; }
    t0 = tick();
    impulses_from_z_and_apply(nic, nib);
    if (pass == 1) { tock(PH_APPLY, t0); break; }
    update_constraint_vels(nic);
    minv = min_cnv(nic);
    bool ch = false;
    double zr = 0.0;
    if (lane < nic) { zr = gd[D_ZSOL + lane] * gd[D_CEPS + gi[I_ISLC + lane]]; ch = zr > MH_NEAR_ZERO; }
    const bool changed = ballot(ch) != 0ull;
    wave_sync();
    if (lane < nic) gd[D_ZBUF + lane] = zr;
    wave_sync();
    bool again = false;
    if (changed) {
      impulses_from_z_and_apply(nic, nib);
      update_constraint_vels(nic);
      const double minv_plus = min_cnv(nic);
      again = (minv_plus < 0.0 && minv_plus < minv - MH_NEAR_ZERO);
    }
    tock(PH_APPLY, t0);
    if (!again) break;
  }
  return false;
}

#if MHW_NOSLIP
MH_DEV bool ns_chol_factor(int n, double* A) {
  for (int j = 0; j < n; j++) {
    double ajj = A[j + n*j];
    for (int k = 0; k < j; k++) ajj = ajj - A[j + n*k] * A[j + n*k];
    if (!(ajj > 0.0)) return false;
    ajj = sqrt(ajj);
    A[j + n*j] = ajj;
    for (int i = j+1; i < n; i++) {
      double t = A[i + n*j];
      for (int k = 0; k < j; k++) t = t - A[i + n*k] * A[j + n*k];
      A[i + n*j] = t / ajj;
    }
  }
  return true;
}
MH_DEV void ns_chol_solve(int n, const double* L, double* b) {
  for (int k = 0; k < n; k++) {
    b[k] = b[k] / L[k + n*k];
    const double bk = b[k];
    for (int i = k+1; i < n; i++) b[i] = b[i] - bk * L[i + n*k];
  }
  for (int k = n-1; k >= 0; k--) {
    double t = b[k];
    for (int i = k+1; i < n; i++) t = t - L[i + n*k] * b[i];
    b[k] = t / L[k + n*k];
  }
}
MH_DEV int ns_build_Y(int nic, int R, int ns, int nt, bool skew) {
  double* Y = gd + D_NSY;
  const int m = ns + nt;
  for (int a = 0; a < ns; a++) for (int b = 0; b < ns; b++) Y[a + m*b] = gd[D_G + (nic + gi[I_NSS + a]) * R + nic + gi[I_NSS + b]];
  for (int a = 0; a < nt; a++) for (int b = 0; b < nt; b++) Y[(ns + a) + m*(ns + b)] = gd[D_G + (2*nic + gi[I_NST + a]) * R + 2*nic + gi[I_NST + b]];
  for (int a = 0; a < ns; a++) for (int b = 0; b < nt; b++) {
    const double g = gd[D_G + (nic + gi[I_NSS + a]) * R + 2*nic + gi[I_NST + b]];
    Y[a + m*(ns + b)] = g; Y[(ns + b) + m*a] = g;
  }
  if (skew) for (int j = 0; j < m; j++) Y[j + m*j] = Y[j + m*j] - MH_NEAR_ZERO;
  return m;
}
MHW_FN int noslip_setup(int nic) {
  nic = uni(nic);
  const int R = 3 * nic;
  wave_sync();
  if (lane_id() == 0) {
    double* Y = gd + D_NSY; double* QX = gd + D_NSQX; double* W = gd + D_NSW; double* col = gd + D_NST2; double* YXv = gd + D_NSYXV;
    int ns = 0, nt = 0;
    for (int i = 0; i < nic; i++) {
      gi[I_NSS + ns] = i; ns++;
      int m = ns_build_Y(nic, R, ns, nt, true);
      if (!ns_chol_factor(m, Y)) ns--;
      gi[I_NST + nt] = i; nt++;
      m = ns_build_Y(nic, R, ns, nt, true);
      if (!ns_chol_factor(m, Y)) nt--;
    }
    const int m = ns_build_Y(nic, R, ns, nt, false);
    int ok = ns_chol_factor(m, Y) ? 1 : 0;
    if (ok) {
      for (int i = 0; i < nic; i++) {
        for (int a = 0; a < ns; a++) QX[i*m + a] = gd[D_G + i * R + nic + gi[I_NSS + a]];
        for (int a = 0; a < nt; a++) QX[i*m + ns + a] = gd[D_G + i * R + 2*nic + gi[I_NST + a]];
      }
      for (int j = 0; j < nic; j++) {
        for (int a = 0; a < m; a++) col[a] = QX[j*m + a];
        ns_chol_solve(m, Y, col);
        for (int a = 0; a < m; a++) W[a + m*j] = col[a];
      }
      for (int i = 0; i < nic; i++) for (int j = 0; j < nic; j++) {
        double acc = 0.0;
        for (int a = 0; a < m; a++) acc = acc + QX[i*m + a] * W[a + m*j];
        gd[D_NSMM + i*nic + j] = gd[D_G + i * R + j] - acc;
      }
      for (int a = 0; a < ns; a++) YXv[a] = gd[D_CV + nic + gi[I_NSS + a]];
      for (int a = 0; a < nt; a++) YXv[ns + a] = gd[D_CV + 2*nic + gi[I_NST + a]];
      ns_chol_solve(m, Y, YXv);
      for (int i = 0; i < nic; i++) {
        double acc = 0.0;
        for (int a = 0; a < m; a++) acc = acc + QX[i*m + a] * YXv[a];
        gd[D_NSQ + i] = gd[D_CV + i] - acc;
      }
    }
    gi[I_NSM] = ok ? m : -1; gi[I_NSNS] = ns;
  }
  wave_sync();
  return geti(I_NSM) >= 0 ? 1 : 0;
}
MHW_FN void noslip_finish(int nic) {
  nic = uni(nic);
  wave_sync();
  if (lane_id() == 0) {
    const int m = gi[I_NSM], ns = gi[I_NSNS], nt = m - ns;
    double* Y = gd + D_NSY; double* QX = gd + D_NSQX; double* t2 = gd + D_NST2; double* YXv = gd + D_NSYXV;
    for (int a = 0; a < m; a++) {
      double acc = 0.0;
      for (int i = 0; i < nic; i++) acc = acc + QX[i*m + a] * gd[D_IMP + i];
      t2[a] = acc;
    }
    ns_chol_solve(m, Y, t2);
    for (int i = 0; i < nic; i++) { gd[D_IMP + nic + i] = 0.0; gd[D_IMP + 2*nic + i] = 0.0; }
    for (int a = 0; a < ns; a++) gd[D_IMP + nic + gi[I_NSS + a]] = -(YXv[a] + t2[a]);
    for (int a = 0; a < nt; a++) gd[D_IMP + 2*nic + gi[I_NST + a]] = -(YXv[ns + a] + t2[ns + a]);
  }
  wave_sync();
}
MH_DEV bool apply_no_slip_model_to_island(int nic, int nib) {
  nic = uni(nic); nib = uni(nib);
  const int lane = lane_id();
  if (3 * nic > MHW_MAX_ROWS || nic > MHW_NS_MAXC) { seti(I_STATUS, geti(I_STATUS) | MH_WORLD_UNSUPPORTED); wave_sync(); return false; }
  unsigned long long t0 = tick();
  compute_problem_data(nic, nib, 3, 0);
  tock(PH_PDATA, t0);
  t0 = tick();
  if (!noslip_setup(nic)) { seti(I_STATUS, geti(I_STATUS) | MH_WORLD_LCP_FAILED); wave_sync(); return true; }
  tock(PH_MBUILD, t0);
  t0 = tick();
  const int n = nic;
  const int zsize = geti(I_VNS_SIZE);
  const double qi = (lane < n) ? gd[D_NSQ + lane] : 0.0;
  double zi = (lane < MH_NOSLIP_MAX) ? gd[D_VNS + lane] : 0.0;
  if (lane >= n) zi = 0.0;
  const ChainOut co = world_lcp_chain(2, nic, n, qi, zi, zsize);
  account(n, uni(co.piv));
  tock(PH_LCP, t0);
  if (!uni(co.ok)) { seti(I_STATUS, geti(I_STATUS) | MH_WORLD_LCP_FAILED); wave_sync(); return true; }
  t0 = tick();
  wave_sync();
  if (lane < n) { gd[D_VNS + lane] = co.zi; gd[D_IMP + lane] = co.zi; }
  seti(I_VNS_SIZE, n);
  noslip_finish(nic);
  apply_impulses(nic, nib, 3);
  update_constraint_vels(nic);
  const double minv = min_cnv(nic);
  bool ch = false; double cn = 0.0;
  if (lane < nic) { cn = gd[D_IMP + lane] * gd[D_CEPS + gi[I_ISLC + lane]]; ch = cn > MH_NEAR_ZERO; }
  const bool changed = ballot(ch) != 0ull;
  wave_sync();
  if (lane < nic) gd[D_IMP + lane] = cn;
  if (changed) {
    if (lane < nic) { gd[D_IMP + nic + lane] = 0.0; gd[D_IMP + 2*nic + lane] = 0.0; }
    wave_sync();
    apply_impulses(nic, nib, 3);
    update_constraint_vels(nic);
    const double minv_plus = min_cnv(nic);
    if (minv_plus < 0.0 && minv_plus < minv - MH_NEAR_ZERO) { seti(I_STATUS, geti(I_STATUS) | MH_WORLD_UNSUPPORTED); }
  }
  wave_sync();
  tock(PH_APPLY, t0);
  return false;
}
#endif

MH_DEV bool thrown() { return (uni(geti(I_STATUS)) & MH_WORLD_LCP_FAILED) != 0; }
MH_DEV bool handle_impacts() {
  const int lane = lane_id();
  const int nc = geti(I_NC);
  if (nc == 0) return false;
  if (ballot(lane < nc && contact_vn(lane) < -MH_NEAR_ZERO) == 0ull) return false;
  islands_begin();
  uint64_t active_contacts = 0;
  while (true) {
    const unsigned long long ti = tick();
    const int isl = next_island();
    tock(PH_ISLANDS, ti);
    if (isl < 0) break;
    const int nic = isl & 0xff, nib = isl >> 8;
    const uint64_t act = ballot(lane < nic && contact_vn(gi[I_ISLC + (lane < nic ? lane : 0)]) < -MH_NEAR_ZERO);
    if (act == 0ull) continue;
    const bool all_inf = ballot(lane < nic && gd[D_CMU + gi[I_ISLC + (lane < nic ? lane : 0)]] < 1e2) == 0ull;
    for (int i = 0; i < nic; i++) active_contacts |= 1ull << geti(I_ISLC + i);
#if MHW_NOSLIP
    if (all_inf) { if (apply_no_slip_model_to_island(nic, nib)) return true; continue; }
#else
    if (all_inf) { seti(I_STATUS, geti(I_STATUS) | MH_WORLD_UNSUPPORTED); wave_sync(); continue; }
#endif
    if (apply_model(nic, nib)) return true;
  }
  if (ballot(lane < nc && ((active_contacts >> lane) & 1ull) && contact_vn(lane) < -MH_NEAR_ZERO) != 0ull) {
    seti(I_STATUS, geti(I_STATUS) | MH_WORLD_IMPACT_TOL); wave_sync();
  }
  return false;
}

MH_DEV void find_unilateral_constraints() {
  const int lane = lane_id();
  const int npairs = geti(I_NPAIRS);
#if MHW_REPORT
  for (int e = lane; e < 3 * MHW_MAX_CONTACTS; e += 64) g_racc[e] = 0.0;
#endif
  ContactGeom c; c.has = 0; c.g1 = 0; c.g2 = 0; c.pt = v3(0, 0, 0); c.n = v3(0, 0, 0); c.dist = 0.0;
  int p = 0;
  const double thresh = gd[D_THRESH];
  bool spk = false;
#if MHW_BOX
  int nc = gen_contacts(I_PAIRS, npairs, 0);
  if (nc < 0) { seti(I_STATUS, geti(I_STATUS) | MH_WORLD_UNSUPPORTED); nc = 0; }
  if (lane < npairs) { int a, b; pair_bodies(gi[I_PAIRS + lane], a, b); spk = is_spokes(a); }
  (void)c; (void)p; (void)thresh;
#else
  if (lane < npairs) {
    p = gi[I_PAIRS + lane];
    int pa_, pb_; pair_bodies(p, pa_, pb_);
    spk = is_spokes(pa_);
    if (!spk) { c = contact_geom(p, thresh); if (c.has && !(c.dist < thresh)) c.has = 0; }
  }
  const uint64_t m = ballot(c.has != 0);
  int nc = popc(m);
  wave_sync();
  if (nc > MHW_MAX_CONTACTS) { seti(I_STATUS, geti(I_STATUS) | MH_WORLD_UNSUPPORTED); nc = 0; }
  else if (c.has) store_contact(popc(m & lanes_below(lane)), p, c.g1, c.g2, c.pt, c.n, c.dist);
#endif
#if MHW_NOSLIP
  { uint64_t sm = ballot(spk);
    while (sm) { const int k = ctz(sm); sm &= sm - 1; nc = spoke_contacts(geti(I_PAIRS + k), nc); } }
#endif
  seti(I_NC, nc);
  wave_sync();
}
#if MHW_NOSLIP
MH_DEV double wheel_ca_loop(double dt) {
  const double min_step = gd[D_MINSTEP];
  const int lane = lane_id();
  double q[7], qs[7], pl[12];
#pragma unroll
  for (int k = 0; k < 7; k++) { q[k] = gd[D_ST + k]; qs[k] = gd[D_QSAVE + k]; }
#pragma unroll
  for (int k = 0; k < 9; k++) pl[k] = gd[D_PLANE_R + k];
#pragma unroll
  for (int k = 0; k < 3; k++) pl[9 + k] = gd[D_PLANE_O + k];
  const int N = geti(I_NSPOKES);
  const double mytx = (lane < MH_MAX_SPOKES) ? gd[D_SPK + 2*lane] : 0.0, mytz = (lane < MH_MAX_SPOKES) ? gd[D_SPK + 2*lane + 1] : 0.0;
  const V3 vl = Vl(0), wa = Wa(0);
  double qd[7];
  { const double nrm = sqrt(((qs[3]*qs[3] + qs[4]*qs[4]) + qs[5]*qs[5]) + qs[6]*qs[6]);
    const double x = qs[3] / nrm, y = qs[4] / nrm, z = qs[5] / nrm, ww = qs[6] / nrm;
    qd[0] = vl.x; qd[1] = vl.y; qd[2] = vl.z;
    qd[3] = 0.5 * ((ww * wa.x + z * wa.y) - y * wa.z);
    qd[4] = 0.5 * ((ww * wa.y + x * wa.z) - z * wa.x);
    qd[5] = 0.5 * ((ww * wa.z + y * wa.x) - x * wa.y);
    qd[6] = 0.5 * (((-x * wa.x) - y * wa.y) - z * wa.z); }
  double h = 0.0;
  unsigned guard = 0;
  while (h < dt) {
    if (++guard > MH_CA_HARD_CAP) { seti(I_STATUS, geti(I_STATUS) | MH_WORLD_STALLED); break; }
    const double x = q[3], y = q[4], z = q[5], w = q[6];
    double R[9];
    R[0] = 1.0 - 2.0 * (y*y + z*z); R[1] = 2.0 * (x*y - z*w);       R[2] = 2.0 * (x*z + y*w);
    R[3] = 2.0 * (x*y + z*w);       R[4] = 1.0 - 2.0 * (x*x + z*z); R[5] = 2.0 * (y*z - x*w);
    R[6] = 2.0 * (x*z - y*w);       R[7] = 2.0 * (y*z + x*w);       R[8] = 1.0 - 2.0 * (x*x + y*y);
    const V3 c = v3(q[0], q[1], q[2]);
    double min_dist; V3 pa, ppm;
    { const double px = mytx, py = 0.0, pz = mytz;
      const V3 tip = v3(c.x + ((R[0]*px + R[1]*py) + R[2]*pz), c.y + ((R[3]*px + R[4]*py) + R[5]*pz), c.z + ((R[6]*px + R[7]*py) + R[8]*pz));
      const V3 d = tip - v3(pl[9], pl[10], pl[11]);
      const V3 pp = v3((pl[0]*d.x + pl[3]*d.y) + pl[6]*d.z, (pl[1]*d.x + pl[4]*d.y) + pl[7]*d.z, (pl[2]*d.x + pl[5]*d.y) + pl[8]*d.z);
      int imin; argmin_first(pp.y, lane < N, min_dist, imin);
      if (imin > 63) { imin = 0; min_dist = MHW_INF; }
      pa = v3(read_lane(tip.x, imin), read_lane(tip.y, imin), read_lane(tip.z, imin));
      ppm = v3(read_lane(pp.x, imin), min_dist, read_lane(pp.z, imin)); }
    double CA = MHW_INF;
    if (!(min_dist <= 0.0)) {
      const V3 pp = v3(ppm.x, 0.0, ppm.z);
      const V3 pb = v3(pl[9] + ((pl[0]*pp.x + pl[1]*pp.y) + pl[2]*pp.z), pl[10] + ((pl[3]*pp.x + pl[4]*pp.y) + pl[5]*pp.z), pl[11] + ((pl[6]*pp.x + pl[7]*pp.y) + pl[8]*pp.z));
      const V3 d0 = pa - pb;
      const V3 n0 = d0 / norm(d0);
      const V3 xd0 = vl + cross(c, wa);
      const double tB = dot(n0, xd0) + norm(cross(wa, n0)) * 0.0;
      double total = 0.0 + tB;
      if (total < 0.0) total = 0.0;
      const double cand = min_dist / total;
      CA = (cand < MHW_INF) ? cand : MHW_INF;
    }
    if (CA <= 0.0) break;
    double tc = (min_step > CA) ? min_step : CA;
    tc = ((dt - h) < tc) ? (dt - h) : tc;
    const double hh = h + tc;
    double qn[7];
#pragma unroll
    for (int k = 0; k < 7; k++) { qn[k] = qd[k] * hh; qn[k] = qn[k] + qs[k]; }
    const double nrm = sqrt(((qn[3]*qn[3] + qn[4]*qn[4]) + qn[5]*qn[5]) + qn[6]*qn[6]);
    q[0] = qn[0]; q[1] = qn[1]; q[2] = qn[2];
    q[3] = qn[3] / nrm; q[4] = qn[4] / nrm; q[5] = qn[5] / nrm; q[6] = qn[6] / nrm;
    h += tc;
  }
  wave_sync();
  if (lane_id() == 0) {
#pragma unroll
    for (int k = 0; k < 7; k++) gd[D_ST + k] = q[k];
    gi[I_PAIRS] = 0; gi[I_NPAIRS] = 1;
  }
  wave_sync();
  return h;
}
#endif

#if MHW_REPORT
MH_DEV void report_fold() {
  const int lane = lane_id();
  double* rep = g_rep;
  const int nc = geti(I_NC);
  wave_sync();
  if (!rep || lane >= gi[I_NPT]) return;
  int a, b; pair_bodies(lane, a, b);
  double* row = rep + MH_REPORT_PAIR * lane;
  for (int c = 0; c < nc; c++) {
    if (gi[I_CPAIR + c] != lane) continue;
    const double cn = g_racc[3*c], cs = g_racc[3*c + 1], ct = g_racc[3*c + 2];
    const V3 n = Cdir(c, 0), s = Cdir(c, 1), t = Cdir(c, 2), pt = Cpt(c);
    const V3 jv = (n * cn + s * cs) + t * ct;
    const double sg = (gi[I_CG1 + c] == a) ? 1.0 : -1.0;
    row[0] = row[0] + 1.0;
    row[1] = row[1] + cn;
    row[2] = row[2] + sg * jv.x; row[3] = row[3] + sg * jv.y; row[4] = row[4] + sg * jv.z;
    row[5] = row[5] + pt.x * cn; row[6] = row[6] + pt.y * cn; row[7] = row[7] + pt.z * cn;
  }
}
#endif

MH_DEV double do_mini_step(double dt, bool& threw) {
  const int lane = lane_id();
  wave_sync();
  if (lane < gi[I_NB]) for (int k = 0; k < 7; k++) gd[D_QSAVE + 7*lane + k] = gd[D_ST + 13*lane + k];
  wave_sync();
  double h = 0.0;
  const double min_step = gd[D_MINSTEP];
#if MHW_NOSLIP
  const bool lone_wheel = geti(I_NB) == 1 && geti(I_NTOT) == 2 && geti(I_GEOM) == MH_GEOM_SPOKES;
  if (lone_wheel) { const unsigned long long tw = tick(); h = uni(wheel_ca_loop(dt)); tock(PH_BROAD_CA, tw); }
  else
#endif
  for (unsigned guard = 0; h < dt; ) {
    if (++guard > MH_CA_HARD_CAP) { seti(I_STATUS, geti(I_STATUS) | MH_WORLD_STALLED); wave_sync(); break; }
    unsigned long long t0 = tick();
    const int npairs = broad_phase(dt - h, I_PAIRS);
    seti(I_NPAIRS, npairs);
    wave_sync();
    const double e = (lane < npairs) ? ca_step(gi[I_PAIRS + lane]) : MHW_INF;
    const double CA = wave_min(e);
    tock(PH_BROAD_CA, t0);
    if (CA <= 0.0) break;
    t0 = tick();
    double tc = (min_step > CA) ? min_step : CA;
    tc = ((dt - h) < tc) ? (dt - h) : tc;
    integrate_positions(h + tc);
    h += tc;
    tock(PH_INTEGRATE, t0);
  }
  unsigned long long t1 = tick();
  integrate_velocities(h);
  tock(PH_FWDDYN, t1);
  t1 = tick();
  find_unilateral_constraints();
  tock(PH_CONTACTS, t1);
  threw = handle_impacts();
  if (threw) return h;
#if MHW_REPORT
  report_fold();
#endif
  if (lane == 0) { gd[D_TIME] = gd[D_TIME] + h; g_cnt[CN_MINI]++; }
  wave_sync();
  return h;
}

struct UniEval { double vmin, uC; };
MHW_FN UniEval eval_unilateral() {
  const int lane = lane_id();
  UniEval r; r.uC = MHW_INF;
  if (lane < geti(I_NPAIRS)) { const PairGeom g = pair_geom(gi[I_PAIRS + lane]); r.uC = g.dist; }
  r.vmin = wave_min(r.uC);
  return r;
}
MH_DEV double eval_at(double t, int idx) {
  set_q_from(D_QV, D_DQV, t, 1);
  const UniEval e = eval_unilateral();
  return read_lane(e.uC, idx);
}
MH_DEV double sign2(double x, double y) { return (y > 0.0) ? fabs(x) : -fabs(x); }
MH_DEV double ridders(double x1, double x2, double fl, double fh, int idx) {
  idx = uni(idx);
  const double TOL = 1e-4;
  double ans = MHW_INF, fm, fnew, s, xh, xl, xm, xnew;
  if ((fl > 0.0 && fh < 0.0) || (fl < 0.0 && fh > 0.0)) {
    xl = x1; xh = x2;
    for (unsigned j = 0; j < 25; j++) {
      xm = 0.5 * (xl + xh);
      fm = eval_at(xm, idx);
      s = sqrt(fm * fm - fl * fh);
      if (s == 0.0) return ans;
      xnew = xm + (xm - xl) * ((fl >= fh ? 1.0 : -1.0) * fm / s);
      ans = xnew;
      fnew = eval_at(ans, idx);
      if (fabs(fnew) < TOL && fnew >= 0.0) return xnew;
      if (sign2(fm, fnew) != fm) { xl = xm; fl = fm; xh = ans; fh = fnew; }
      else if (sign2(fl, fnew) != fl) { xh = ans; fh = fnew; }
      else if (sign2(fh, fnew) != fh) { xl = ans; fl = fnew; }
    }
  } else {
    if (fl == 0.0) return x1;
    if (fh == 0.0) return x2;
  }
  return 0.0;
}
MH_DEV int update_q() {
  const int lane = lane_id();
  const int npairs = geti(I_NPAIRS);
  const double uC_old = eval_unilateral().uC;
  set_q_from(D_QV, D_DQV, 1.0, 0);
  double uC = eval_unilateral().uC;
  const bool br = (lane < npairs) && ((uC_old < 0.0 && uC > 0.0) || (uC_old > 0.0 && uC < 0.0));
  const uint64_t brm = ballot(br);
  double t = 1.0;
  { uint64_t m = brm;
    while (m) {
      const int i = ctz(m); m &= m - 1;
      const double root = uni(ridders(0.0, t, read_lane(uC_old, i), read_lane(uC, i), i));
      if (root > 0.0 && root < 1.0) t = (root < t) ? root : t;
    } }
  set_q_from(D_QV, D_DQV, t, 1);
  uC = eval_unilateral().uC;
  const double BETA = 0.6;
  while (true) {
    const bool bad = (lane < npairs) && !br && uC < 0.0 && uC_old > uC;
    if (ballot(bad) == 0ull) break;
    t *= BETA;
    if (t < MH_NEAR_ZERO) return 0;
    set_q_from(D_QV, D_DQV, t, 1);
    uC = eval_unilateral().uC;
  }
  wave_sync();
  if (lane < gi[I_NB]) for (int k = 0; k < 7; k++) { const double v = gd[D_DQV + 7*lane + k] * t; gd[D_QV + 7*lane + k] = v + gd[D_QV + 7*lane + k]; }
  wave_sync();
  return 1;
}
MHW_FN void stabilize_work(double max_uvio) {
  const int lane = lane_id();
  const unsigned max_it = (unsigned)geti(I_CSTAB_MAXIT);
  const int nb = geti(I_NB);
  const double cstab_eps = gd[D_CSTABEPS];
  wave_sync();
  if (lane < nb) {
    for (int k = 0; k < 6; k++) gd[D_VSAVE + 6*lane + k] = gd[D_ST + 13*lane + 7 + k];
    for (int k = 0; k < 7; k++) gd[D_QV + 7*lane + k] = gd[D_ST + 13*lane + k];
  }
  wave_sync();
  unsigned iterations = 0;
  while (max_uvio < cstab_eps) {
    if (iterations == max_it) break;
    if (iterations == MH_CSTAB_HARD_CAP) { seti(I_STATUS, geti(I_STATUS) | MH_WORLD_STALLED); wave_sync(); break; }
    wave_sync();
    if (lane < nb) { for (int k = 0; k < 6; k++) gd[D_ST + 13*lane + 7 + k] = 0.0; for (int k = 0; k < 7; k++) gd[D_DQV + 7*lane + k] = 0.0; }
    wave_sync();
    const int ncp = broad_phase(0.0, I_SCR);
    ContactGeom c; c.has = 0; c.g1 = 0; c.g2 = 0; c.pt = v3(0, 0, 0); c.n = v3(0, 0, 0); c.dist = 0.0;
    int p = 0;
    bool spk = false;
    PairGeom g; g.dist = 0.0; g.a = 0; g.b = 0; g.pa = v3(0, 0, 0); g.pb = v3(0, 0, 0);
#if MHW_BOX
    int nc = gen_contacts(I_SCR, ncp, 1);
    if (nc < 0) { seti(I_STATUS, geti(I_STATUS) | MH_WORLD_UNSUPPORTED); seti(I_NC, 0); wave_sync(); break; }
    if (lane < ncp) { p = gi[I_SCR + lane]; int a, b; pair_bodies(p, a, b); spk = is_spokes(a); if (spk) g = pair_geom(p); }
    (void)c;
#else
    if (lane < ncp) {
      p = gi[I_SCR + lane];
      g = pair_geom(p);
      spk = is_spokes(g.b);
      if (spk) { }
      else if (g.dist >= MH_NEAR_ZERO) {
        const V3 nn = g.pb - g.pa;
        c.n = nn / norm(nn); c.pt = g.pa; c.g1 = g.a; c.g2 = g.b; c.dist = g.dist; c.has = 1;
      } else c = contact_geom(p, MH_NEAR_ZERO);
    }
    const uint64_t m = ballot(c.has != 0);
    int nc = popc(m);
    wave_sync();
    if (nc > MHW_MAX_CONTACTS) { seti(I_STATUS, geti(I_STATUS) | MH_WORLD_UNSUPPORTED); seti(I_NC, 0); wave_sync(); break; }
    if (c.has) store_contact(popc(m & lanes_below(lane)), p, c.g1, c.g2, c.pt, c.n, c.dist);
#endif
#if MHW_NOSLIP
    { uint64_t sm = ballot(spk);
      bool over = false;
      while (sm) {
        const int k = ctz(sm); sm &= sm - 1;
        const double dk = read_lane(g.dist, k);
        if (dk >= MH_NEAR_ZERO) {
          if (nc >= MHW_MAX_CONTACTS) { over = true; break; }
          wave_sync();
          if (lane == k) { const V3 nn = g.pb - g.pa; store_contact(nc, p, g.a, g.b, g.pa, nn / norm(nn), g.dist); }
          wave_sync();
          nc++;
        } else nc = spoke_contacts(geti(I_SCR + k), nc);
      }
      if (over) { seti(I_STATUS, geti(I_STATUS) | MH_WORLD_UNSUPPORTED); seti(I_NC, 0); wave_sync(); break; } }
#endif
    seti(I_NC, nc);
    wave_sync();
    islands_begin();
    while (true) {
      const int isl = next_island();
      if (isl < 0) break;
      const int nic = isl & 0xff, nib = isl >> 8;
      const int n_ = nic;
      if (n_ > MHW_MAX_ROWS) { seti(I_STATUS, geti(I_STATUS) | MH_WORLD_UNSUPPORTED); wave_sync(); continue; }
      compute_problem_data(nic, nib, 1, 1);
      if (n_ > geti(I_NMAX)) { seti(I_STATUS, geti(I_STATUS) | MH_WORLD_UNSUPPORTED); wave_sync(); continue; }
      double qi = 0.0;
      if (lane < n_) qi = gd[D_CDIST + gi[I_ISLC + lane]] - fabs(cstab_eps) - MH_NEAR_ZERO;
      wave_sync();
      const ChainOut co = world_lcp_chain(1, nic, n_, qi, 0.0, 0);
      const double zi = co.zi; const int zsize = uni(co.zsize);
      account(n_, uni(co.piv)); if (lane_id() == 0) g_cnt[CN_SROWS] += (unsigned long long)n_;
      wave_sync();
      if (lane < n_) gd[D_IMP + lane] = (lane < zsize) ? zi : 0.0;
      wave_sync();
      apply_impulses(nic, nib, 1);
      if (lane < nib) { const int b = gi[I_ISLB + lane]; double qd[7]; euler_vel(b, qd); for (int k = 0; k < 7; k++) gd[D_DQV + 7*b + k] = qd[k]; }
      wave_sync();
    }
    if (!update_q()) { seti(I_STATUS, geti(I_STATUS) | MH_WORLD_STAB_FAILED); wave_sync(); break; }
    max_uvio = eval_unilateral().vmin;
    iterations++;
    if (lane == 0) g_cnt[CN_STAB]++;
  }
  wave_sync();
  if (lane < nb) for (int k = 0; k < 6; k++) gd[D_ST + 13*lane + 7 + k] = gd[D_VSAVE + 6*lane + k];
  wave_sync();
}

MH_DEV void stabilize() {
  if (geti(I_CSTAB_MAXIT) == 0) return;
  const double max_uvio = eval_unilateral().vmin;
  if (!(max_uvio < gd[D_CSTABEPS])) return;
  stabilize_work(max_uvio);
}

MH_DEV bool world_step(double dt) {
  seti(I_NPAIRS, broad_phase(dt, I_PAIRS));
  wave_sync();
  double h = 0.0;
  unsigned guard = 0;
  while (h < dt) {
    bool threw = false;
    h += uni(do_mini_step(dt - h, threw));
    if (threw) return true;
    if (++guard > 100000u) { seti(I_STATUS, geti(I_STATUS) | MH_WORLD_STALLED); wave_sync(); break; }
  }
  const unsigned long long ts = tick();
  stabilize();
  tock(PH_STAB, ts);
  if (lane_id() == 0) g_cnt[CN_STEPS]++;
  return false;
}

__global__ __launch_bounds__(64, MHW_WAVES_PER_SIMD)
void mh_k_world_step(const mh_scene* __restrict__ scp, int B, double dt, int nsteps, double* __restrict__ state,
                     mh_world_aux* __restrict__ aux, double* __restrict__ traj, int nmax, double* __restrict__ lu_ws, int ka,
                     unsigned long long* __restrict__ prof, const int* __restrict__ ids
#if MHW_FORCES
                     , const mh_world_forces* __restrict__ frc, const double* __restrict__ wrench, int wrows
#endif
#if MHW_REPORT
                     , double* __restrict__ report
#endif
                     )
{
  const int w = ids ? ids[blockIdx.x] : (int)blockIdx.x;
  if ((unsigned)w >= (unsigned)B) return;
  const int lane = lane_id();
  const mh_scene& sc = *scp;
#if MHW_STATICS
  const mh_world_statics& sst = *reinterpret_cast<const mh_world_statics*>(reinterpret_cast<const double*>(scp + 1) + 2 * MH_MAX_SPOKES);
#endif
#if MHW_PARAMS
  static_assert((sizeof(mh_scene) + 2 * MH_MAX_SPOKES * sizeof(double) + sizeof(mh_world_statics)) % 8 == 0 && sizeof(mh_world_params) % 8 == 0, "params records must be 8-byte aligned");
  const mh_world_params& pv = reinterpret_cast<const mh_world_params*>(&sst + 1)[w];
#define MHW_ST_R(k) pv.st_R[k]
#define MHW_ST_O(k) pv.st_o[k]
#define MHW_ST_DIM(k) pv.st_dim[k]
#else
  const mh_scene& pv = sc;
#define MHW_ST_R(k) sst.R[k]
#define MHW_ST_O(k) sst.o[k]
#define MHW_ST_DIM(k) sst.dim[k]
#endif
#if MHW_STATICS
  const int hg = sc.has_ground ? 1 : 0, nst_ = sst.n;
  const int nb = sc.nb, ntot = sc.nb + hg + nst_, npt = ntot * (ntot - 1) / 2;
  if (nb < 1 || nst_ < 0 || ntot > MH_MAX_BODIES + 1) return;
  if (lane < hg + nst_) {
    const int k = lane - hg;
    const bool gr = k < 0;
    gst[lane] = gr ? MH_STATIC_PLANE : sst.type[k];
    for (int q = 0; q < 9; q++) gs[S_R + 9*lane + q] = gr ? pv.plane_R[q] : MHW_ST_R(k)[q];
    for (int q = 0; q < 3; q++) gs[S_O + 3*lane + q] = gr ? pv.plane_o[q] : MHW_ST_O(k)[q];
    const double x = gr ? 0.0 : MHW_ST_DIM(k)[0], y = gr ? 0.0 : MHW_ST_DIM(k)[1], z = gr ? 0.0 : MHW_ST_DIM(k)[2];
    gs[S_DIM + 3*lane] = x; gs[S_DIM + 3*lane + 1] = y; gs[S_DIM + 3*lane + 2] = z;
    const double hx = x / 2.0, hy = y / 2.0, hz = z / 2.0;
    gs[S_RAD + lane] = sqrt((hx*hx + hy*hy) + hz*hz);
  } else if (lane < MH_MAX_STATICS) gst[lane] = -1;
#else
  const int nb = sc.nb, ntot = sc.nb + (sc.has_ground ? 1 : 0), npt = ntot * (ntot - 1) / 2;
#endif
  if (lane < nb) {
    gi[I_GEOM + lane] = sc.geom_type[lane];
    { const int gt = sc.geom_type[lane];
      const double x = pv.geom_dim[lane][0], y = pv.geom_dim[lane][1], z = pv.geom_dim[lane][2];
      double rad = 0.0, rmax = 0.0;
      if (gt == MH_GEOM_SPHERE) { rad = x; rmax = x; }
      else if (gt == MH_GEOM_BOX) {
        const double hx = x / 2.0, hy = y / 2.0, hz = z / 2.0;
        rad = sqrt((hx*hx + hy*hy) + hz*hz); rmax = sqrt((x*x + y*y) + z*z);
      }
      gd[D_RADIUS + lane] = rad; gd[D_RMAX + lane] = rmax;
#if MHW_BOX
      gd[D_GDIM + 3*lane] = x; gd[D_GDIM + 3*lane + 1] = y; gd[D_GDIM + 3*lane + 2] = z;
#endif
    }
    gd[D_MASS + lane] = pv.mass[lane];
    for (int k = 0; k < 3; k++) gd[D_INERTIA + 3*lane + k] = pv.inertia[lane][k];
  }
  if (lane < 9) gd[D_PLANE_R + lane] = pv.plane_R[lane];
  if (lane < 3) { gd[D_PLANE_O + lane] = pv.plane_o[lane]; gd[D_GRAV + lane] = pv.gravity[lane]; }
  if (lane < npt) {
    gd[D_PMU + lane] = pv.cp_mu_coulomb[lane]; gd[D_PMUV + lane] = pv.cp_mu_viscous[lane];
    gd[D_PEPS + lane] = pv.cp_epsilon[lane]; gd[D_PCOMP + lane] = pv.cp_compliance[lane];
    gi[I_PNK + lane] = sc.cp_nk[lane]; gi[I_PEN + lane] = sc.pair_enabled[lane];
  }
#if MHW_FORCES
  { const int ft = frc ? frc->terms : 0;
    if (lane < nb) {
      const bool st = (ft & MH_FORCE_STOKES) != 0, dm = (ft & MH_FORCE_DAMPING) != 0;
      gf[F_SB + lane] = st ? frc->stokes_b[lane] : 0.0; gf[F_SBA + lane] = st ? frc->stokes_b_ang[lane] : 0.0;
      gf[F_KL + lane] = dm ? frc->damp_kl[lane] : 0.0; gf[F_KA + lane] = dm ? frc->damp_ka[lane] : 0.0;
      gf[F_KLSQ + lane] = dm ? frc->damp_klsq[lane] : 0.0; gf[F_KASQ + lane] = dm ? frc->damp_kasq[lane] : 0.0;
    }
    if (lane == 0) g_fterms = (ft & (MH_FORCE_STOKES | MH_FORCE_DAMPING)) | (wrench ? MHW_FORCE_WRENCH : 0); }
#endif
  mh_world_aux* a = aux + w;
  if (lane == 0) {
    gd[D_MINSTEP] = sc.min_step_size; gd[D_THRESH] = sc.contact_dist_thresh; gd[D_CSTABEPS] = sc.cstab_eps; gd[D_TIME] = a->time;
    gi[I_NB] = nb; gi[I_NTOT] = ntot; gi[I_NPT] = npt; gi[I_NMAX] = nmax; gi[I_KA] = (ka < MHW_KA_V) ? ka : MHW_KA_V; gi[I_NPAIRS] = 0; gi[I_NC] = 0;
    gi[I_STATUS] = a->status; gi[I_ZLAST_SIZE] = a->zlast_size; gi[I_ZBUF_SIZE] = a->zbuf_size; gi[I_ZBUF_CAP] = a->zbuf_cap;
    gi[I_NODEMASK] = 0; gi[I_DONEMASK] = 0; gi[I_DONEMASK_HI] = 0; gi[I_CSTAB_MAXIT] = (int)sc.cstab_max_iterations;
    gi[I_NSPOKES] = 0; gi[I_VNS_SIZE] = a->vns_size; gi[I_NSM] = 0; gi[I_NSNS] = 0;
    for (int b = 0; b < nb; b++) if (sc.geom_type[b] == MH_GEOM_SPOKES) gi[I_NSPOKES] = (int)sc.geom_dim[b][1];
    g_lu_ws = lu_ws + (size_t)w * nmax * nmax;
    g_cnt[CN_STEPS] = a->steps; g_cnt[CN_MINI] = a->mini_steps; g_cnt[CN_LCP] = a->lcp_solves; g_cnt[CN_ROWS] = a->lcp_rows;
    g_cnt[CN_PIV] = a->lcp_pivots; g_cnt[CN_STAB] = a->stab_iters; g_cnt[CN_BYTES] = a->lcp_alg_bytes; g_cnt[CN_SROWS] = a->stab_rows;
    for (int i = 0; i < PH_COUNT; i++) g_pacc[i] = 0ull;
    g_lcp_prof_on = prof ? 1 : 0; for (int i = 0; i < LP_COUNT; i++) g_lcp_prof[i] = 0ull;
  }
  const int nst = MH_BODY_STATE * nb;
  double* stg = state + (size_t)w * nst;
  for (int e = lane; e < nst; e += 64) gd[D_ST + e] = stg[e];
  if (lane < 32) gi[I_RNG + lane] = (int)a->rng[lane];
  gd[D_ZLAST + lane] = a->zlast[lane]; gd[D_ZBUF + lane] = a->zbuf[lane];
  if (lane < 4 * nb) gd[D_XQ + lane] = __longlong_as_double(0x7ff8000000000000ll);
#if MHW_NOSLIP
  { const double* spk = reinterpret_cast<const double*>(scp + 1);
    if (lane < 2 * MH_MAX_SPOKES) gd[D_SPK + lane] = spk[lane];
    if (lane < MH_NOSLIP_MAX) gd[D_VNS + lane] = a->vns[lane]; }
#endif
  wave_sync();
  bool dead = thrown();
  for (int s = 0; s < nsteps; s++) {
#if MHW_FORCES
    if (wrench && !dead && (s == 0 || wrows > 1)) {
      wave_sync();
      if (lane < 6 * nb) gf[F_WR + lane] = wrench[((size_t)(wrows > 1 ? s : 0) * B + w) * (size_t)(6 * nb) + lane];
      wave_sync();
    }
#endif
#if MHW_REPORT
    wave_sync();
    { double* rows = report ? report + ((size_t)w * nsteps + s) * (size_t)npt * MH_REPORT_PAIR : nullptr;
      if (lane == 0) g_rep = rows;
      if (rows && lane < npt) for (int k = 0; k < MH_REPORT_PAIR; k++) rows[MH_REPORT_PAIR * lane + k] = 0.0; }
    wave_sync();
#endif
    if (!dead) dead = world_step(dt);
    if (traj) {
      wave_sync();
      for (int e = lane; e < 7 * nb; e += 64) { const int b = e / 7, k = e - 7 * b; traj[(((size_t)w * nsteps + s) * nb + b) * 7 + k] = gd[D_ST + 13 * b + k]; }
    }
  }
  wave_sync();
  for (int e = lane; e < nst; e += 64) stg[e] = gd[D_ST + e];
  if (lane < 32) a->rng[lane] = (uint32_t)gi[I_RNG + lane];
  a->zlast[lane] = gd[D_ZLAST + lane]; a->zbuf[lane] = gd[D_ZBUF + lane];
#if MHW_NOSLIP
  if (lane < MH_NOSLIP_MAX) a->vns[lane] = gd[D_VNS + lane];
  if (lane == 0) a->vns_size = gi[I_VNS_SIZE];
#endif
  if (lane == 0) {
    a->zlast_size = gi[I_ZLAST_SIZE]; a->zbuf_size = gi[I_ZBUF_SIZE]; a->zbuf_cap = gi[I_ZBUF_CAP]; a->status = gi[I_STATUS]; a->time = gd[D_TIME];
    a->steps = g_cnt[CN_STEPS]; a->mini_steps = g_cnt[CN_MINI]; a->lcp_solves = g_cnt[CN_LCP]; a->lcp_rows = g_cnt[CN_ROWS];
    a->lcp_pivots = g_cnt[CN_PIV]; a->stab_iters = g_cnt[CN_STAB]; a->lcp_alg_bytes = g_cnt[CN_BYTES]; a->stab_rows = g_cnt[CN_SROWS];
    if (prof) { for (int i = 0; i < LP_COUNT; i++) g_pacc[PH_LP0 + i] = g_lcp_prof[i]; for (int i = 0; i < PH_COUNT; i++) prof[(size_t)w * PH_COUNT + i] = g_pacc[i]; }
  }
}

#undef MHW_FN
#undef MHW_ST_R
#undef MHW_ST_O
#undef MHW_ST_DIM
#undef plane_body
#undef box_plane_pair
} }

#if MHW_FORCES
#define MHW_FORCES_ARGS(a) , (a).forces, (a).wrench, (a).wrench_rows
#else
#define MHW_FORCES_ARGS(a)
#endif
#if MHW_REPORT
#define MHW_REPORT_ARGS(a) , (a).report
#else
#define MHW_REPORT_ARGS(a)
#endif
static hipError_t launch(const mh_world_launch& a)
{
  hipLaunchKernelGGL(mh::MHW_NS::mh_k_world_step, dim3(a.grid), dim3(64), 0, a.stream,
                     a.scene, a.B, a.dt, a.nsteps, a.state, a.aux, a.traj, a.nmax, a.lu_ws, a.ka, a.prof, a.ids MHW_FORCES_ARGS(a) MHW_REPORT_ARGS(a));
  return hipGetLastError();
}
static hipError_t occupancy(int* blocks_per_cu)
{
  return hipOccupancyMaxActiveBlocksPerMultiprocessor(blocks_per_cu, mh::MHW_NS::mh_k_world_step, 64, 0);
}
static hipError_t upload_tables(const void* fric, size_t fric_bytes, const void* pow10, size_t pow10_bytes)
{
  if (fric_bytes != sizeof(mh::FricTable) || pow10_bytes != sizeof(mh::Pow10Table)) return hipErrorInvalidValue;
  hipError_t e = hipMemcpyToSymbol(HIP_SYMBOL(mh::c_fric), fric, fric_bytes);
  if (e == hipSuccess) e = hipMemcpyToSymbol(HIP_SYMBOL(mh::c_pow10), pow10, pow10_bytes);
  return e;
}

const mh_world_variant* MHW_VARIANT_GETTER()
{
  static const mh_world_variant v = { launch, occupancy, mh::MHW_NS::PH_COUNT, upload_tables };
  return &v;
}
```

Baseline: 2.314 billion.

## Keep island, contact-count and friction-offset state in registers instead of LDS

Replaces LDS-stored island search state, contact counts and pair counts with values passed through registers. Friction-direction offsets are now computed by a wave-parallel prefix (packed into a 64-bit register for small islands) instead of a serial lane-0 loop. The matrix norm is folded into the G-matrix build, and gc_of is replaced by a bitmask popcount. The broad phase at the start of world_step is skipped in most cases. Together these cut redundant LDS round-trips, wave syncs and serial loops, at the cost of extra register pressure and more complex index logic.

```diff
diff --git a/moby_amd/csrc/mh_lcp_wave.h b/moby_amd/csrc/mh_lcp_wave.h
--- a/moby_amd/csrc/mh_lcp_wave.h
+++ b/moby_amd/csrc/mh_lcp_wave.h
@@ -8,8 +8,11 @@
 __shared__ unsigned long long g_lcp_prof[LP_COUNT];
 __shared__ int g_lcp_prof_on;
 #ifdef MH_PROFILE_BUILD
+MH_DEV void lds_add(unsigned long long* p, unsigned long long v) {
+  if (lane_id() == 0) (void)__hip_atomic_fetch_add(p, v, __ATOMIC_RELAXED, __HIP_MEMORY_SCOPE_WAVEFRONT);
+}
 MH_DEV unsigned long long lp_tick() { return g_lcp_prof_on ? __builtin_amdgcn_s_memtime() : 0ull; }
-MH_DEV void lp_tock(int ph, unsigned long long t0) { if (g_lcp_prof_on) { const unsigned long long d = __builtin_amdgcn_s_memtime() - t0; if (lane_id() == 0) g_lcp_prof[ph] += d; } }
+MH_DEV void lp_tock(int ph, unsigned long long t0) { if (g_lcp_prof_on) { const unsigned long long d = __builtin_amdgcn_s_memtime() - t0; lds_add(&g_lcp_prof[ph], d); } }
 #else
 MH_DEV unsigned long long lp_tick() { return 0ull; }
 MH_DEV void lp_tock(int, unsigned long long) {}
diff --git a/moby_amd/csrc/mh_world_wave.inc b/moby_amd/csrc/mh_world_wave.inc
--- a/moby_amd/csrc/mh_world_wave.inc
+++ b/moby_amd/csrc/mh_world_wave.inc
@@ -128,13 +128,14 @@
 MH_DEV void seti(int i, int v) { if (lane_id() == 0) gi[i] = v; }
 #ifdef MH_PROFILE_BUILD
 MH_DEV unsigned long long tick() { return g_lcp_prof_on ? __builtin_amdgcn_s_memtime() : 0ull; }
-MH_DEV void tock(int ph, unsigned long long t0) { if (g_lcp_prof_on) { const unsigned long long d = __builtin_amdgcn_s_memtime() - t0; if (lane_id() == 0) g_pacc[ph] += d; } }
+MH_DEV void tock(int ph, unsigned long long t0) { if (g_lcp_prof_on) { const unsigned long long d = __builtin_amdgcn_s_memtime() - t0; lds_add(&g_pacc[ph], d); } }
 #else
 MH_DEV unsigned long long tick() { return 0ull; }
 MH_DEV void tock(int, unsigned long long) {}
 #endif
+MH_DEV void count(int c, unsigned long long v) { if (lane_id() == 0) g_cnt[c] += v; }
 MH_DEV void account(int n, unsigned piv) {
-  if (lane_id() == 0) { g_cnt[CN_LCP]++; g_cnt[CN_ROWS] += (unsigned long long)n; g_cnt[CN_PIV] += piv; g_cnt[CN_BYTES] += 8ull * ((unsigned long long)n * n + 2ull * n); }
+  count(CN_LCP, 1ull); count(CN_ROWS, (unsigned long long)n); count(CN_PIV, piv); count(CN_BYTES, 8ull * ((unsigned long long)n * n + 2ull * n));
 }
 
 MH_DEV bool enabled(int b) { return b < gi[I_NB]; }
@@ -798,32 +799,35 @@
 }
 #endif
 
-MH_DEV void islands_begin() {
-  const int lane = lane_id();
-  const int nc = geti(I_NC), nb = geti(I_NB);
+struct IslandSearch { unsigned node_mask; uint64_t done; };
+struct Island { int nic, nib; unsigned bodies; uint64_t contacts; };
+MH_DEV IslandSearch islands_begin(int nc) {
+  nc = uni(nc);
+  const int lane = lane_id();
+  const int nb = geti(I_NB);
   const bool in = lane < nc;
   const int a = in ? gi[I_CG1 + lane] : -1, b = in ? gi[I_CG2 + lane] : -1;
   unsigned nodes = 0;
   for (int k = 0; k < nb; k++) if (ballot(in && (a == k || b == k)) != 0ull) nodes |= 1u << k;
-  wave_sync();
-  seti(I_NODEMASK, (int)nodes); seti(I_DONEMASK, 0); seti(I_DONEMASK_HI, 0);
-  wave_sync();
-}
-MH_DEV int next_island() {
-  const int lane = lane_id();
-  const int nc = geti(I_NC);
-  unsigned node_mask = (unsigned)geti(I_NODEMASK);
-  uint64_t done = (uint64_t)(unsigned)geti(I_DONEMASK) | ((uint64_t)(unsigned)geti(I_DONEMASK_HI) << 32);
+  IslandSearch s; s.node_mask = nodes; s.done = 0ull;
+  return s;
+}
+MH_DEV bool next_island(int nc, IslandSearch& s, Island& isl) {
+  nc = uni(nc);
+  const int lane = lane_id();
+  unsigned node_mask = s.node_mask;
+  uint64_t done = s.done;
   const bool in = lane < nc;
   const int a = in ? gi[I_CG1 + lane] : -1, b = in ? gi[I_CG2 + lane] : -1;
   const uint64_t both = ballot(in && enabled(a) && enabled(b));
-  int result = -1;
+  bool found = false;
   wave_sync();
   while (node_mask) {
     const int start = __ffs((int)node_mask) - 1;
     unsigned visited = 1u << start, bodies = 0;
     uint64_t queue = (uint64_t)start; int qlen = 1;
     int nic = 0;
+    uint64_t contacts = 0ull;
     while (qlen > 0) {
       const int nd = (int)(queue & 15ull); queue >>= 4; qlen--;
       node_mask &= ~(1u << nd);
@@ -839,22 +843,22 @@
       const uint64_t fresh = touch & ~done;
       if ((fresh >> lane) & 1ull) gi[I_ISLC + nic + popc(fresh & lanes_below(lane))] = lane;
       nic += popc(fresh);
-      done |= fresh;
+      done |= fresh; contacts |= fresh;
     }
     if (nic == 0) continue;
     if (lane < 32 && ((bodies >> lane) & 1u)) gi[I_ISLB + popc((uint64_t)(bodies & ((1u << lane) - 1u)))] = lane;
-    result = nic | (popc((uint64_t)bodies) << 8);
+    isl.nic = nic; isl.nib = popc((uint64_t)bodies); isl.bodies = bodies; isl.contacts = contacts;
+    found = true;
     break;
   }
   wave_sync();
-  seti(I_NODEMASK, (int)node_mask); seti(I_DONEMASK, (int)(unsigned)done); seti(I_DONEMASK_HI, (int)(unsigned)(done >> 32));
-  wave_sync();
-  return result;
-}
-
-MH_DEV int gc_of(int body, int nib) { for (int k = 0; k < nib; k++) if (gi[I_ISLB + k] == body) return 6 * k; return -1; }
-MH_DEV void compute_problem_data(int nic, int nib, int ndir, int fresh_xinv) {
-  nic = uni(nic); nib = uni(nib); ndir = uni(ndir); fresh_xinv = uni(fresh_xinv);
+  s.node_mask = node_mask; s.done = done;
+  return found;
+}
+
+MH_DEV int gc_of(int body, unsigned bodies) { return ((bodies >> body) & 1u) ? 6 * popc((uint64_t)(bodies & ((1u << body) - 1u))) : -1; }
+MH_DEV double compute_problem_data(int nic, unsigned bodies, int ndir, int fresh_xinv, bool want_norm) {
+  nic = uni(nic); bodies = uni(bodies); ndir = uni(ndir); fresh_xinv = uni(fresh_xinv);
   const int lane = lane_id();
   const int R = ndir * nic;
   if (fresh_xinv) compute_xinv();
@@ -871,7 +875,7 @@
       const V3 dd = (k == 0) ? dir : -dir;
       const V3 r = pt - X(b);
       const V3 rxd = cross(r, dd);
-      gi[I_ROWOFF + 2*lane + k] = gc_of(b, nib);
+      gi[I_ROWOFF + 2*lane + k] = gc_of(b, bodies);
       Jr[0] = dd.x; Jr[1] = dd.y; Jr[2] = dd.z; Jr[3] = rxd.x; Jr[4] = rxd.y; Jr[5] = rxd.z;
       const double im = gd[D_XINV + 10*b]; const double* Ji = gd + D_XINV + 10*b + 1;
       XJr[0] = dd.x * im; XJr[1] = dd.y * im; XJr[2] = dd.z * im;
@@ -886,10 +890,12 @@
     gd[D_CV + lane] = cv;
   }
   wave_sync();
+  double nmax = 0.0;
   {
     const unsigned mnic = small_div_magic(nic), mR = small_div_magic(R);
     for (int e = lane; e < R * R; e += 64) {
       int r = small_div_m(e, mR), c = e - r * R;
+      const bool ndiag = (r == c) && (r < nic);
       if (small_div_m(c, mnic) < small_div_m(r, mnic)) { const int t = r; r = c; c = t; }
       double res = 0.0;
 #pragma unroll
@@ -907,18 +913,51 @@
         res = res + tmp;
       }
       gd[D_G + e] = res;
-    }
-  }
-  wave_sync();
-}
-
+      if (want_norm) {
+        double g = res;
+        if (ndiag) g = g + gd[D_CCOMP + gi[I_ISLC + r]];
+        const double a = fabs(g); nmax = (a > nmax) ? a : nmax;
+      }
+    }
+  }
+  if (want_norm) {
+    if (lane < nic) { const double a = fabs(gd[D_CMU + gi[I_ISLC + lane]]); nmax = (a > nmax) ? a : nmax; }
+    nmax = wave_max(nmax);
+    nmax = (nmax > 1.0) ? nmax : 1.0;
+  }
+  wave_sync();
+  return nmax;
+}
+
+struct PolyIndex { int total; uint64_t pack; int ri, rbase; };
+enum { POLY_PACK = 7 };
+MH_DEV int poly_koff(uint64_t pack, int i) { return (int)((pack >> (8 * i)) & 0xffull); }
+MH_DEV PolyIndex poly_index(int nic) {
+  const int lane = lane_id();
+  const int cnk = (lane < nic) ? gi[I_CNK + gi[I_ISLC + lane]] / 2 : 0;
+  const int rr = lane - 6 * nic;
+  PolyIndex x; x.pack = 0ull; x.ri = 0; x.rbase = 0;
+  int off = 0, total = 0;
+  for (int k = 0; k < nic; k++) {
+    const int ck = read_lane(cnk, k);
+    if (lane > k) off += ck;
+    total += ck;
+    if (k < POLY_PACK) x.pack |= (uint64_t)(unsigned)total << (8 * (k + 1));
+    if (k + 1 < nic && rr >= total) { x.ri = k + 1; x.rbase = total; }
+  }
+  if (nic > POLY_PACK && lane <= nic) gi[I_KOFF + lane] = off;
+  x.total = total;
+  return x;
+}
 struct WorldMat {
   int mode, nic, R, nvars, n, doff; unsigned mnic;
+  uint64_t kpack;
   int rkind, ra, ri, grow, gcol, rneg, rvar;
   double rmu, rcos, rsin, rcomp;
+  double nrm;
   MH_DEV static int dir_of(int a) { return (a == 0) ? 0 : ((a == 1 || a == 3) ? 1 : 2); }
-  MH_DEV void init(int mode_, int nic_, int n_) {
-    mode = mode_; nic = nic_; n = n_;
+  MH_DEV void init(int mode_, int nic_, int n_, double nrm_, const PolyIndex& px) {
+    mode = mode_; nic = nic_; n = n_; nrm = nrm_; kpack = uni(px.pack);
     doff = (mode == 2) ? (int)D_NSMM : (int)D_G;
     R = (mode == 0) ? 3 * nic_ : nic_; nvars = 5 * nic_; mnic = 0u;
     const int r = lane_id();
@@ -930,8 +969,8 @@
     else if (r < n) {
       rkind = 2;
       const int rr = r - nvars - nic;
-      int i = 0; while (rr >= gi[I_KOFF + i + 1]) i++;
-      ri = i; const int rj = rr - gi[I_KOFF + i];
+      const int i = px.ri;
+      ri = i; const int rj = rr - px.rbase;
       const int ci = gi[I_ISLC + i]; const int kh = gi[I_CNK + ci] / 2;
       rmu = gd[D_CMU + ci]; rcos = c_fric.c[kh][rj]; rsin = c_fric.s[kh][rj];
     }
@@ -962,9 +1001,11 @@
       if (ra == 0 && ri == cc) g = g + rcomp;
       return -g;
     }
-    int i = 0; const int rr = cc - nic; while (rr >= gi[I_KOFF + i + 1]) i++;
+    int i = 0, k0; const int rr = cc - nic;
+    if (nic <= POLY_PACK) { while (rr >= poly_koff(kpack, i + 1)) i++; k0 = poly_koff(kpack, i); }
+    else { while (rr >= gi[I_KOFF + i + 1]) i++; k0 = gi[I_KOFF + i]; }
     if (i != ri) return -0.0;
-    const int jj = rr - gi[I_KOFF + i]; const int ci = gi[I_ISLC + i]; const int kh = gi[I_CNK + ci] / 2;
+    const int jj = rr - k0; const int ci = gi[I_ISLC + i]; const int kh = gi[I_CNK + ci] / 2;
     const double v = (ra == 0) ? gd[D_CMU + ci] : ((ra == 1 || ra == 3) ? -c_fric.c[kh][jj] : -c_fric.s[kh][jj]);
     return -v;
   }
@@ -976,21 +1017,11 @@
     return g;
   }
   MH_DEV double norm_all() const {
+    if (mode == 0) return nrm;
     const int lane = lane_id();
     double m = 0.0;
-    if (mode != 0) {
-      if (lane < n) for (int c = 0; c < n; c++) { const double a = fabs(gd[doff + lane * n + c]); m = (a > m) ? a : m; }
-      return wave_max(m);
-    }
-    for (int e = lane; e < R * R; e += 64) {
-      const int r = small_div(e, R), c = e - r * R;
-      double g = gd[D_G + e];
-      if (r == c && r < nic) g = g + gd[D_CCOMP + gi[I_ISLC + r]];
-      const double a = fabs(g); m = (a > m) ? a : m;
-    }
-    if (lane < nic) { const double a = fabs(gd[D_CMU + gi[I_ISLC + lane]]); m = (a > m) ? a : m; }
-    m = wave_max(m);
-    return (m > 1.0) ? m : 1.0;
+    if (lane < n) for (int c = 0; c < n; c++) { const double a = fabs(gd[doff + lane * n + c]); m = (a > m) ? a : m; }
+    return wave_max(m);
   }
   MH_DEV double offdiag_max() const {
     if (mode != 0) {
@@ -998,17 +1029,17 @@
       if (lane < n) for (int c = 0; c < n; c++) { const double a = fabs(gd[doff + lane * n + c]); if (c != lane && a > m) m = a; }
       return wave_max(m);
     }
-    return norm_all();
+    return nrm;
   }
 };
 
 struct ChainOut { int ok; double zi; int zsize; unsigned piv; };
-MH_DEV ChainOut world_lcp_chain(int mode, int nic, int n, double qi, double zi, int zsize)
+MH_DEV ChainOut world_lcp_chain(int mode, int nic, int n, double qi, double zi, int zsize, double nrm, const PolyIndex& px)
 {
-  mode = uni(mode); nic = uni(nic); n = uni(n); zsize = uni(zsize);
+  mode = uni(mode); nic = uni(nic); n = uni(n); zsize = uni(zsize); nrm = uni(nrm);
   const int lane = lane_id();
   const unsigned long long ts = lp_tick();
-  WorldMat M; M.init(mode, nic, n);
+  WorldMat M; M.init(mode, nic, n, nrm, px);
   const double nrm0 = M.norm_all(), dii = M.diag();
   lp_tock(LP_SETUP, ts);
   WaveRand rng; rng.r = (lane < 31) ? (unsigned)gi[I_RNG + lane] : 0u; rng.idx = geti(I_RNG + 31);
@@ -1039,13 +1070,12 @@
   return o;
 }
 
-MH_DEV int solve_impact_lcp(int nic) {
+MH_DEV int solve_impact_lcp(int nic, double nrm) {
   nic = uni(nic);
   const int lane = lane_id();
-  wave_sync();
-  if (lane == 0) { int acc = 0; for (int i = 0; i < nic; i++) { gi[I_KOFF + i] = acc; acc += gi[I_CNK + gi[I_ISLC + i]] / 2; } gi[I_KOFF + nic] = acc; }
-  wave_sync();
-  const int nk_total = geti(I_KOFF + nic);
+  const PolyIndex px = poly_index(nic);
+  wave_sync();
+  const int nk_total = px.total;
   const int nvars = 5 * nic, n = nvars + nic + nk_total;
   if (n > geti(I_NMAX) || n > MH_LCP_MAX_N_WAVE) { seti(I_STATUS, geti(I_STATUS) | MH_WORLD_UNSUPPORTED); wave_sync(); return 0; }
   unsigned long long tm = tick();
@@ -1055,7 +1085,7 @@
     if (r < nvars) { const int a = small_div(r, nic), i = r - a * nic; const double v = gd[D_CV + WorldMat::dir_of(a) * nic + i]; qi = (a >= 3) ? -v : v; }
     else if (r < nvars + nic) qi = gd[D_CV + r - nvars];
     else {
-      int i = 0; const int rr = r - nvars - nic; while (rr >= gi[I_KOFF + i + 1]) i++;
+      const int i = px.ri;
       const double cs = gd[D_CV + nic + i], ct = gd[D_CV + 2 * nic + i];
       const double vel = sqrt(cs * cs + ct * ct);
       qi = gd[D_CMUV + gi[I_ISLC + i]] * vel;
@@ -1068,7 +1098,7 @@
   if (n > zbuf_cap) zi = 0.0; else zi = gd[D_ZBUF + lane];
   if (lane >= n) zi = 0.0;
   if (n == zlast_size) zi = (lane < n) ? gd[D_ZLAST + lane] : 0.0;
-  const ChainOut co = world_lcp_chain(0, nic, n, qi, zi, n);
+  const ChainOut co = world_lcp_chain(0, nic, n, qi, zi, n, nrm, px);
   zi = co.zi;
   const bool ok = uni(co.ok) != 0;
   account(n, uni(co.piv));
@@ -1149,16 +1179,16 @@
 }
 MH_DEV double min_cnv(int nic) { const int lane = lane_id(); return wave_min((lane < nic) ? gd[D_CV + lane] : MHW_INF); }
 
-MH_DEV bool apply_model(int nic, int nib) {
-  nic = uni(nic); nib = uni(nib);
+MH_DEV bool apply_model(const Island& isl) {
+  const int nic = uni(isl.nic), nib = uni(isl.nib);
   const int lane = lane_id();
   if (3 * nic > MHW_MAX_ROWS) { seti(I_STATUS, geti(I_STATUS) | MH_WORLD_UNSUPPORTED); wave_sync(); return false; }
   unsigned long long t0 = tick();
-  compute_problem_data(nic, nib, 3, 0);
+  const double nrm = compute_problem_data(nic, isl.bodies, 3, 0, true);
   tock(PH_PDATA, t0);
   double minv = 0.0;
   for (int pass = 0; pass < 2; pass++) {
-    { const int rs = solve_impact_lcp(nic); if (rs <= 0) return rs < 0; }
+    { const int rs = solve_impact_lcp(nic, nrm); if (rs <= 0) return rs < 0; }
     t0 = tick();
     impulses_from_z_and_apply(nic, nib);
     if (pass == 1) { tock(PH_APPLY, t0); break; }
@@ -1288,12 +1318,12 @@
   }
   wave_sync();
 }
-MH_DEV bool apply_no_slip_model_to_island(int nic, int nib) {
-  nic = uni(nic); nib = uni(nib);
+MH_DEV bool apply_no_slip_model_to_island(const Island& isl) {
+  const int nic = uni(isl.nic), nib = uni(isl.nib);
   const int lane = lane_id();
   if (3 * nic > MHW_MAX_ROWS || nic > MHW_NS_MAXC) { seti(I_STATUS, geti(I_STATUS) | MH_WORLD_UNSUPPORTED); wave_sync(); return false; }
   unsigned long long t0 = tick();
-  compute_problem_data(nic, nib, 3, 0);
+  compute_problem_data(nic, isl.bodies, 3, 0, false);
   tock(PH_PDATA, t0);
   t0 = tick();
   if (!noslip_setup(nic)) { seti(I_STATUS, geti(I_STATUS) | MH_WORLD_LCP_FAILED); wave_sync(); return true; }
@@ -1304,7 +1334,7 @@
   const double qi = (lane < n) ? gd[D_NSQ + lane] : 0.0;
   double zi = (lane < MH_NOSLIP_MAX) ? gd[D_VNS + lane] : 0.0;
   if (lane >= n) zi = 0.0;
-  const ChainOut co = world_lcp_chain(2, nic, n, qi, zi, zsize);
+  const ChainOut co = world_lcp_chain(2, nic, n, qi, zi, zsize, 0.0, PolyIndex());
   account(n, uni(co.piv));
   tock(PH_LCP, t0);
   if (!uni(co.ok)) { seti(I_STATUS, geti(I_STATUS) | MH_WORLD_LCP_FAILED); wave_sync(); return true; }
@@ -1336,29 +1366,30 @@
 #endif
 
 MH_DEV bool thrown() { return (uni(geti(I_STATUS)) & MH_WORLD_LCP_FAILED) != 0; }
-MH_DEV bool handle_impacts() {
-  const int lane = lane_id();
-  const int nc = geti(I_NC);
+MH_DEV bool handle_impacts(int nc) {
+  nc = uni(nc);
+  const int lane = lane_id();
   if (nc == 0) return false;
-  if (ballot(lane < nc && contact_vn(lane) < -MH_NEAR_ZERO) == 0ull) return false;
-  islands_begin();
+  const uint64_t impacting = ballot(lane < nc && contact_vn(lane) < -MH_NEAR_ZERO);
+  if (impacting == 0ull) return false;
+  IslandSearch search = islands_begin(nc);
   uint64_t active_contacts = 0;
   while (true) {
     const unsigned long long ti = tick();
-    const int isl = next_island();
+    Island isl;
+    const bool more = next_island(nc, search, isl);
     tock(PH_ISLANDS, ti);
-    if (isl < 0) break;
-    const int nic = isl & 0xff, nib = isl >> 8;
-    const uint64_t act = ballot(lane < nic && contact_vn(gi[I_ISLC + (lane < nic ? lane : 0)]) < -MH_NEAR_ZERO);
-    if (act == 0ull) continue;
+    if (!more) break;
+    const int nic = isl.nic;
+    if ((impacting & isl.contacts) == 0ull) continue;
     const bool all_inf = ballot(lane < nic && gd[D_CMU + gi[I_ISLC + (lane < nic ? lane : 0)]] < 1e2) == 0ull;
-    for (int i = 0; i < nic; i++) active_contacts |= 1ull << geti(I_ISLC + i);
+    active_contacts |= isl.contacts;
 #if MHW_NOSLIP
-    if (all_inf) { if (apply_no_slip_model_to_island(nic, nib)) return true; continue; }
+    if (all_inf) { if (apply_no_slip_model_to_island(isl)) return true; continue; }
 #else
     if (all_inf) { seti(I_STATUS, geti(I_STATUS) | MH_WORLD_UNSUPPORTED); wave_sync(); continue; }
 #endif
-    if (apply_model(nic, nib)) return true;
+    if (apply_model(isl)) return true;
   }
   if (ballot(lane < nc && ((active_contacts >> lane) & 1ull) && contact_vn(lane) < -MH_NEAR_ZERO) != 0ull) {
     seti(I_STATUS, geti(I_STATUS) | MH_WORLD_IMPACT_TOL); wave_sync();
@@ -1366,9 +1397,9 @@
   return false;
 }
 
-MH_DEV void find_unilateral_constraints() {
-  const int lane = lane_id();
-  const int npairs = geti(I_NPAIRS);
+MH_DEV int find_unilateral_constraints(int npairs) {
+  npairs = uni(npairs);
+  const int lane = lane_id();
 #if MHW_REPORT
   for (int e = lane; e < 3 * MHW_MAX_CONTACTS; e += 64) g_racc[e] = 0.0;
 #endif
@@ -1398,8 +1429,8 @@
   { uint64_t sm = ballot(spk);
     while (sm) { const int k = ctz(sm); sm &= sm - 1; nc = spoke_contacts(geti(I_PAIRS + k), nc); } }
 #endif
-  seti(I_NC, nc);
-  wave_sync();
+  wave_sync();
+  return nc;
 }
 #if MHW_NOSLIP
 MH_DEV double wheel_ca_loop(double dt) {
@@ -1471,7 +1502,7 @@
   if (lane_id() == 0) {
 #pragma unroll
     for (int k = 0; k < 7; k++) gd[D_ST + k] = q[k];
-    gi[I_PAIRS] = 0; gi[I_NPAIRS] = 1;
+    gi[I_PAIRS] = 0;
   }
   wave_sync();
   return h;
@@ -1479,10 +1510,9 @@
 #endif
 
 #if MHW_REPORT
-MH_DEV void report_fold() {
+MH_DEV void report_fold(int nc) {
   const int lane = lane_id();
   double* rep = g_rep;
-  const int nc = geti(I_NC);
   wave_sync();
   if (!rep || lane >= gi[I_NPT]) return;
   int a, b; pair_bodies(lane, a, b);
@@ -1501,6 +1531,13 @@
 }
 #endif
 
+MH_DEV bool lone_wheel() {
+#if MHW_NOSLIP
+  return geti(I_NB) == 1 && geti(I_NTOT) == 2 && geti(I_GEOM) == MH_GEOM_SPOKES;
+#else
+  return false;
+#endif
+}
 MH_DEV double do_mini_step(double dt, bool& threw) {
   const int lane = lane_id();
   wave_sync();
@@ -1508,17 +1545,15 @@
   wave_sync();
   double h = 0.0;
   const double min_step = gd[D_MINSTEP];
+  int npairs = 0;
 #if MHW_NOSLIP
-  const bool lone_wheel = geti(I_NB) == 1 && geti(I_NTOT) == 2 && geti(I_GEOM) == MH_GEOM_SPOKES;
-  if (lone_wheel) { const unsigned long long tw = tick(); h = uni(wheel_ca_loop(dt)); tock(PH_BROAD_CA, tw); }
+  if (lone_wheel()) { const unsigned long long tw = tick(); h = uni(wheel_ca_loop(dt)); tock(PH_BROAD_CA, tw); npairs = 1; }
   else
 #endif
   for (unsigned guard = 0; h < dt; ) {
     if (++guard > MH_CA_HARD_CAP) { seti(I_STATUS, geti(I_STATUS) | MH_WORLD_STALLED); wave_sync(); break; }
     unsigned long long t0 = tick();
-    const int npairs = broad_phase(dt - h, I_PAIRS);
-    seti(I_NPAIRS, npairs);
-    wave_sync();
+    npairs = broad_phase(dt - h, I_PAIRS);
     const double e = (lane < npairs) ? ca_step(gi[I_PAIRS + lane]) : MHW_INF;
     const double CA = wave_min(e);
     tock(PH_BROAD_CA, t0);
@@ -1530,18 +1565,20 @@
     h += tc;
     tock(PH_INTEGRATE, t0);
   }
+  seti(I_NPAIRS, npairs);
   unsigned long long t1 = tick();
   integrate_velocities(h);
   tock(PH_FWDDYN, t1);
   t1 = tick();
-  find_unilateral_constraints();
+  const int nc = find_unilateral_constraints(npairs);
   tock(PH_CONTACTS, t1);
-  threw = handle_impacts();
+  threw = handle_impacts(nc);
   if (threw) return h;
 #if MHW_REPORT
-  report_fold();
-#endif
-  if (lane == 0) { gd[D_TIME] = gd[D_TIME] + h; g_cnt[CN_MINI]++; }
+  report_fold(nc);
+#endif
+  if (lane == 0) gd[D_TIME] = gd[D_TIME] + h;
+  count(CN_MINI, 1ull);
   wave_sync();
   return h;
 }
@@ -1641,7 +1678,7 @@
     PairGeom g; g.dist = 0.0; g.a = 0; g.b = 0; g.pa = v3(0, 0, 0); g.pb = v3(0, 0, 0);
 #if MHW_BOX
     int nc = gen_contacts(I_SCR, ncp, 1);
-    if (nc < 0) { seti(I_STATUS, geti(I_STATUS) | MH_WORLD_UNSUPPORTED); seti(I_NC, 0); wave_sync(); break; }
+    if (nc < 0) { seti(I_STATUS, geti(I_STATUS) | MH_WORLD_UNSUPPORTED); wave_sync(); break; }
     if (lane < ncp) { p = gi[I_SCR + lane]; int a, b; pair_bodies(p, a, b); spk = is_spokes(a); if (spk) g = pair_geom(p); }
     (void)c;
 #else
@@ -1658,7 +1695,7 @@
     const uint64_t m = ballot(c.has != 0);
     int nc = popc(m);
     wave_sync();
-    if (nc > MHW_MAX_CONTACTS) { seti(I_STATUS, geti(I_STATUS) | MH_WORLD_UNSUPPORTED); seti(I_NC, 0); wave_sync(); break; }
+    if (nc > MHW_MAX_CONTACTS) { seti(I_STATUS, geti(I_STATUS) | MH_WORLD_UNSUPPORTED); wave_sync(); break; }
     if (c.has) store_contact(popc(m & lanes_below(lane)), p, c.g1, c.g2, c.pt, c.n, c.dist);
 #endif
 #if MHW_NOSLIP
@@ -1675,25 +1712,24 @@
           nc++;
         } else nc = spoke_contacts(geti(I_SCR + k), nc);
       }
-      if (over) { seti(I_STATUS, geti(I_STATUS) | MH_WORLD_UNSUPPORTED); seti(I_NC, 0); wave_sync(); break; } }
-#endif
-    seti(I_NC, nc);
+      if (over) { seti(I_STATUS, geti(I_STATUS) | MH_WORLD_UNSUPPORTED); wave_sync(); break; } }
+#endif
     wave_sync();
-    islands_begin();
+    IslandSearch search = islands_begin(nc);
     while (true) {
-      const int isl = next_island();
-      if (isl < 0) break;
-      const int nic = isl & 0xff, nib = isl >> 8;
+      Island isl;
+      if (!next_island(nc, search, isl)) break;
+      const int nic = isl.nic, nib = isl.nib;
       const int n_ = nic;
       if (n_ > MHW_MAX_ROWS) { seti(I_STATUS, geti(I_STATUS) | MH_WORLD_UNSUPPORTED); wave_sync(); continue; }
-      compute_problem_data(nic, nib, 1, 1);
+      compute_problem_data(nic, isl.bodies, 1, 1, false);
       if (n_ > geti(I_NMAX)) { seti(I_STATUS, geti(I_STATUS) | MH_WORLD_UNSUPPORTED); wave_sync(); continue; }
       double qi = 0.0;
       if (lane < n_) qi = gd[D_CDIST + gi[I_ISLC + lane]] - fabs(cstab_eps) - MH_NEAR_ZERO;
       wave_sync();
-      const ChainOut co = world_lcp_chain(1, nic, n_, qi, 0.0, 0);
+      const ChainOut co = world_lcp_chain(1, nic, n_, qi, 0.0, 0, 0.0, PolyIndex());
       const double zi = co.zi; const int zsize = uni(co.zsize);
-      account(n_, uni(co.piv)); if (lane_id() == 0) g_cnt[CN_SROWS] += (unsigned long long)n_;
+      account(n_, uni(co.piv)); count(CN_SROWS, (unsigned long long)n_);
       wave_sync();
       if (lane < n_) gd[D_IMP + lane] = (lane < zsize) ? zi : 0.0;
       wave_sync();
@@ -1704,7 +1740,7 @@
     if (!update_q()) { seti(I_STATUS, geti(I_STATUS) | MH_WORLD_STAB_FAILED); wave_sync(); break; }
     max_uvio = eval_unilateral().vmin;
     iterations++;
-    if (lane == 0) g_cnt[CN_STAB]++;
+    count(CN_STAB, 1ull);
   }
   wave_sync();
   if (lane < nb) for (int k = 0; k < 6; k++) gd[D_ST + 13*lane + 7 + k] = gd[D_VSAVE + 6*lane + k];
@@ -1719,8 +1755,7 @@
 }
 
 MH_DEV bool world_step(double dt) {
-  seti(I_NPAIRS, broad_phase(dt, I_PAIRS));
-  wave_sync();
+  if (lone_wheel() || !(0.0 < dt)) { seti(I_NPAIRS, broad_phase(dt, I_PAIRS)); wave_sync(); }
   double h = 0.0;
   unsigned guard = 0;
   while (h < dt) {
@@ -1732,7 +1767,7 @@
   const unsigned long long ts = tick();
   stabilize();
   tock(PH_STAB, ts);
-  if (lane_id() == 0) g_cnt[CN_STEPS]++;
+  count(CN_STEPS, 1ull);
   return false;
 }
 
@@ -1823,9 +1858,9 @@
   mh_world_aux* a = aux + w;
   if (lane == 0) {
     gd[D_MINSTEP] = sc.min_step_size; gd[D_THRESH] = sc.contact_dist_thresh; gd[D_CSTABEPS] = sc.cstab_eps; gd[D_TIME] = a->time;
-    gi[I_NB] = nb; gi[I_NTOT] = ntot; gi[I_NPT] = npt; gi[I_NMAX] = nmax; gi[I_KA] = (ka < MHW_KA_V) ? ka : MHW_KA_V; gi[I_NPAIRS] = 0; gi[I_NC] = 0;
+    gi[I_NB] = nb; gi[I_NTOT] = ntot; gi[I_NPT] = npt; gi[I_NMAX] = nmax; gi[I_KA] = (ka < MHW_KA_V) ? ka : MHW_KA_V; gi[I_NPAIRS] = 0;
     gi[I_STATUS] = a->status; gi[I_ZLAST_SIZE] = a->zlast_size; gi[I_ZBUF_SIZE] = a->zbuf_size; gi[I_ZBUF_CAP] = a->zbuf_cap;
-    gi[I_NODEMASK] = 0; gi[I_DONEMASK] = 0; gi[I_DONEMASK_HI] = 0; gi[I_CSTAB_MAXIT] = (int)sc.cstab_max_iterations;
+    gi[I_CSTAB_MAXIT] = (int)sc.cstab_max_iterations;
     gi[I_NSPOKES] = 0; gi[I_VNS_SIZE] = a->vns_size; gi[I_NSM] = 0; gi[I_NSNS] = 0;
     for (int b = 0; b < nb; b++) if (sc.geom_type[b] == MH_GEOM_SPOKES) gi[I_NSPOKES] = (int)sc.geom_dim[b][1];
     g_lu_ws = lu_ws + (size_t)w * nmax * nmax;
```

Result: faster. 2.431 billion, median of 6 (+5.1%).
